# mahfuzalhasan/WaveFormer

Hardware: AMD Instinct MI355X
Metric: 128³×4 volumes/sec fwd (1/2/4/8 MI355X) + Dice Δ vs reference (higher is better)
Workload: dtype bf16x3; 1 GPU; MultiscaleTransformer (WaveFormer encoder) forward, 128^3x4 crops; global_batch=8, per_gpu_batch=8, precision=bf16x3, parallelism=replicas x1 (no data-path collective), hip_graph=True

## Files before the change

include/waveformer_hip.h:

```cpp
#ifndef WAVEFORMER_HIP_H
#define WAVEFORMER_HIP_H

#include <stdint.h>

#ifdef __cplusplus
extern "C" {
#endif

#define WF_ABI_VERSION 20

enum { WF_PREC_BF16 = 0, WF_PREC_BF16X3 = 1, WF_PREC_FP16 = 2 };

enum {
  WF_OK = 0,
  WF_E_SHAPE = -1,
  WF_E_NULLPTR = -2,
  WF_E_LAUNCH = -3
};

int wf_abi_version(void);
const char* wf_last_error(void);


int wf_cast_f32_to_bf16(const float* in, uint16_t* out, int64_t n, void* stream);

int wf_split_f32_to_bf16x2(const float* in, uint16_t* out, int64_t n, void* stream);

int wf_split_f32_to_bf16x2_multi(const int64_t* table_dev, int64_t n, int64_t total,
                                 void* stream);

int wf_cast_f32_to_f16x2(const float* in, uint16_t* out, int64_t n, void* stream);
int wf_cast_f32_to_f16x2_multi(const int64_t* table_dev, int64_t n, int64_t total,
                               void* stream);

int wf_debug_poison_lds(int64_t blocks, int lds_bytes, void* stream);

int wf_patch_embed_fwd(const float* x, const float* w, const float* bias, float* out,
                       int64_t B, int64_t Cin, int64_t Cout, int64_t D, int64_t H, int64_t W,
                       void* stream);
int wf_patch_embed_ll_fwd(const float* x, const float* w, const float* bias, float* out,
                          const float* ln_w, const float* ln_b, float ln_eps, float* ll,
                          int64_t B, int64_t Cin, int64_t Cout, int64_t D, int64_t H, int64_t W,
                          void* stream);

int wf_dwt3d_haar_fwd(const float* x, const float* ln_w, const float* ln_b, float ln_eps,
                      float* bands, int64_t B, int64_t C, int64_t D, int64_t H, int64_t W,
                      void* stream);
int wf_dwt3d_haar_fwd_ll(const float* x, const float* ln_w, const float* ln_b, float ln_eps,
                         float* ll, int64_t B, int64_t C, int64_t D, int64_t H, int64_t W,
                         void* stream);

int wf_idwt3d_haar(const float* ll, int64_t ll_bstride, const float* const* det,
                   const int64_t* det_s, int levels, float* out, int64_t out_bstride,
                   int64_t B, int64_t C, int64_t d, int64_t h, int64_t w, void* stream);
int wf_idwt3d_haar_cl(const float* ll, int64_t ll_bstride, int64_t ll_cstride,
                      int64_t ll_pstride, const float* const* det, const int64_t* det_s,
                      int levels, float* out, int64_t out_bstride, int64_t ldo, int64_t B,
                      int64_t C, int64_t d, int64_t h, int64_t w, void* stream);

int wf_idwt3d_haar_cl_cat(const float* ll, int64_t ll_bstride, int64_t ll_cstride,
                          int64_t ll_pstride, const float* const* det, const int64_t* det_s,
                          int levels, const float* skip, int64_t skip_bstride, int64_t skip_ld,
                          float* out, int64_t out_bstride, int64_t ldo, int64_t B, int64_t C,
                          int64_t d, int64_t h, int64_t w, void* stream);

int wf_copy_cl(const float* src, int64_t lds, float* dst, int64_t ldd, int64_t P, int64_t C,
               void* stream);
int wf_subvoxel_scatter_cl(const float* g, const float* bias, float* dst, int64_t ldd,
                           int64_t B, int64_t C, int64_t d, int64_t h, int64_t w, void* stream);
int wf_convtranspose2_cl(const float* x, const uint16_t* w_bf16x2, const float* bias, float* out,
                         int64_t ldo, int64_t B, int64_t Cin, int64_t Cout, int64_t d, int64_t h,
                         int64_t w, int precision, void* stream);

int wf_dwt3d_fwd(const float* x, float* bands, int64_t P, int64_t D, int64_t H, int64_t W,
                 const float* dec_lo, const float* dec_hi, int taps, void* stream);

int wf_idwt3d_level(const float* const* coef, const int64_t* coef_strides, int64_t B, int64_t C,
                    int64_t n_z, int64_t n_y, int64_t n_x, const float* rec_lo,
                    const float* rec_hi, int taps, float* out, int64_t out_bstride,
                    int64_t out_cstride, void* stream);

int wf_dwt3d_bwd(const float* gbands, float* dx, int64_t P, int64_t D, int64_t H, int64_t W,
                 const float* dec_lo, const float* dec_hi, int taps, void* stream);

int wf_idwt3d_level_bwd(const float* gout, int64_t gout_bstride, int64_t gout_cstride, int64_t B,
                        int64_t C, int64_t n_z, int64_t n_y, int64_t n_x, int extra_z,
                        int extra_y, int extra_x, const float* rec_lo, const float* rec_hi,
                        int taps, float* const* gcoef, const int64_t* gcoef_strides,
                        void* stream);

int64_t wf_conv3d_k3_packed_elems(int64_t Cin, int64_t Cout);
int wf_conv3d_k3_pack(const float* w, uint16_t* packed, int64_t Cin, int64_t Cout, void* stream);
int wf_conv3d_k3_pack_f16(const float* w, uint16_t* packed, int64_t Cin, int64_t Cout,
                          void* stream);
int64_t wf_conv3d_k3_workspace_bytes(int64_t B, int64_t Cin, int64_t Cout, int64_t D, int64_t H,
                                     int64_t W, int precision, int fp16_input);
int wf_conv3d_k3_fwd(const float* x, int64_t ldx, const uint16_t* w_packed, const float* bias,
                     float* out, int64_t ldo, double* stats_acc, void* workspace, int64_t B,
                     int64_t Cin, int64_t Cout, int64_t D, int64_t H, int64_t W, int precision,
                     void* stream);
int wf_conv3d_k3_fwd_xh(const uint16_t* x, int64_t ldx, const uint16_t* w_packed_f16,
                        const float* bias, float* out, int64_t ldo, double* stats_acc,
                        void* workspace, int64_t B, int64_t Cin, int64_t Cout, int64_t D,
                        int64_t H, int64_t W, void* stream);

int64_t wf_conv3d_k3_wgrad_workspace_bytes(int64_t B, int64_t Cin, int64_t Cout, int64_t D,
                                           int64_t H, int64_t W);
int wf_conv3d_k3_wgrad(const float* x, int64_t ldx, const float* dy, int64_t ldg, float* dw,
                       int accumulate, void* workspace, int64_t B, int64_t Cin, int64_t Cout,
                       int64_t D, int64_t H, int64_t W, void* stream);

int64_t wf_instnorm_workspace_bytes(int64_t B, int64_t C);
int wf_instnorm_stats_cl(const float* x, int64_t ldx, int64_t B, int64_t C, int64_t P, float eps,
                         float* stats, void* workspace, void* stream);
int wf_instnorm_finalize(const double* acc, float* stats, int64_t B, int64_t C, int64_t P,
                         float eps, void* stream);
int wf_norm_act_cl(const float* a, int64_t lda, const float* stats_a, const float* r, int64_t ldr,
                   const float* stats_r, float* out, int64_t ldo, int64_t B, int64_t C, int64_t P,
                   float slope, void* stream);
int wf_norm_act_h_cl(const float* a, int64_t lda, const float* stats_a, uint16_t* out,
                     int64_t ldo, int64_t B, int64_t C, int64_t P, float slope, void* stream);

int wf_moments_cl(const float* x, int64_t ldx, int64_t B, int64_t K, int64_t P, double* acc,
                  void* stream);
int wf_norm_act_lin_cl(const float* a, int64_t lda, const float* stats_a, const float* x,
                       int64_t ldx, int64_t K, const float* wfold, const float* bfold,
                       float* out, int64_t ldo, int64_t B, int64_t C, int64_t P, float slope,
                       void* stream);

int64_t wf_hf_refine_workspace_bytes(int64_t B, int64_t C);
int wf_hf_refine_fwd(const float* const* details, int64_t ldb, const float* dw_w,
                     const float* dw_b, const float* in_w, const float* in_b, float eps,
                     const float* pw_w, const float* pw_b, int sigmoid, float* out,
                     void* workspace, int64_t B, int64_t C, int64_t D, int64_t H, int64_t W,
                     void* stream);

int64_t wf_norm_act_bwd_workspace_bytes(int64_t B, int64_t C);
int wf_norm_act_bwd_cl(const float* dy, int64_t ldd, const float* y, int64_t ldy,
                       const float* a, int64_t lda, const float* stats_a, const float* r,
                       int64_t ldr, const float* stats_r, float* da, int64_t ldda, float* dr,
                       int64_t lddr, int64_t B, int64_t C, int64_t P, float slope,
                       void* workspace, void* stream);

int wf_upsample_trilinear_cl(const float* in, float* out, int64_t B, int64_t C, int64_t d,
                             int64_t h, int64_t w, int64_t D, int64_t H, int64_t W,
                             int align_corners, void* stream);
int wf_upsample_trilinear_add_cl(const float* in, float* out, int64_t B, int64_t C, int64_t d,
                                 int64_t h, int64_t w, int64_t D, int64_t H, int64_t W,
                                 int align_corners, void* stream);
int wf_upsample_dwconv3d_stats_cl(const float* in, const float* w, const float* bias, float* out,
                                  double* stats_acc, int64_t B, int64_t C, int64_t d, int64_t h,
                                  int64_t wd, int64_t D, int64_t H, int64_t W, int align_corners,
                                  void* stream);
int wf_conv1x1_head_cl(const float* x, int64_t ldx, const float* weight, const float* bias,
                       float* out, int64_t B, int64_t K, int64_t N, int64_t P, void* stream);
int wf_linear_smallk_fwd(const float* x, int64_t ldx, const float* w, const float* bias,
                         float* y, int64_t ldy, int64_t M, int64_t K, int64_t N, void* stream);
int wf_dwconv3d_stats_cl(const float* in, const float* w, const float* bias, float* out,
                         double* stats_acc, int64_t B, int64_t C, int64_t D, int64_t H,
                         int64_t W, void* stream);

int wf_resample_trilinear_cf(const float* in, int64_t ldc, int64_t C, int64_t d, int64_t h,
                             int64_t w, int64_t D, int64_t H, int64_t W, int align_corners,
                             void* out, int out_f16, void* stream);

int wf_linear_fwd(const float* x, const uint16_t* w_bf16x2, const float* bias, float* out,
                  int64_t M, int64_t K, int64_t N, int gelu_in, int precision, void* stream);

int wf_window_attention_fwd_table(const float* x, const float* ln_w, const float* ln_b,
                                  float ln_eps, const uint16_t* wqkv_bf16x2, const float* bqkv,
                                  const float* table, const uint16_t* wproj_bf16x2,
                                  const float* bproj, float* out, void* workspace, int64_t B,
                                  int64_t C, int64_t D1, int64_t H1, int64_t W1, int64_t ws,
                                  int64_t heads, float scale, int precision, void* stream);

int wf_rel_pos_bias(const float* table, const int64_t* index, float* bias, int64_t N,
                    int64_t heads, int64_t table_rows, void* stream);

int64_t wf_window_attention_workspace_bytes(int64_t B, int64_t C, int64_t D1, int64_t H1,
                                            int64_t W1, int precision);
int wf_window_attention_fwd(const float* x, const float* ln_w, const float* ln_b, float ln_eps,
                            const uint16_t* wqkv_bf16x2, const float* bqkv,
                            const float* bias, const uint16_t* wproj_bf16x2, const float* bproj,
                            float* out, void* workspace, int64_t B, int64_t C, int64_t D1,
                            int64_t H1, int64_t W1, int64_t ws, int64_t heads, float scale,
                            int precision, void* stream);

int64_t wf_window_attention_levels_workspace_bytes(const int64_t* dhw, int nlev, int64_t B,
                                                   int64_t C, int precision);
int wf_window_attention_fwd_levels(const float* const* x, const int64_t* dhw, int nlev,
                                   const uint16_t* wqkv_bf16x2, const float* bqkv,
                                   const float* table, const uint16_t* wproj_bf16x2,
                                   const float* bproj, float* out, void* workspace, int64_t B,
                                   int64_t C, int64_t heads, float scale, int precision,
                                   void* stream);

int wf_msfuse_fwd(const float* const* src, const int64_t* src_dhw, int nsrc,
                  const float* shortcut, const float* branch_scale, float* out, float* stats,
                  float ln_eps, int64_t B, int64_t C, int64_t D, int64_t H, int64_t W,
                  void* stream);

int64_t wf_ccf_ffn_workspace_bytes(int64_t B, int64_t C, int64_t hidden, int64_t D, int64_t H,
                                   int64_t W, int precision);
int wf_ccf_ffn_fwd(const float* xh, const float* stats, const float* n2_w, const float* n2_b,
                   const uint16_t* pw_bf16x2, const float* pw_b, const float* ln1_w,
                   const float* ln1_b, float eps1, const float* dw_w, const float* dw_b,
                   const float* ln2_w, const float* ln2_b, float eps2,
                   const uint16_t* fc_bf16x2, const float* fc_b, const float* branch_scale,
                   float* out, void* workspace,
                   int64_t B, int64_t C, int64_t hidden, int64_t D, int64_t H, int64_t W,
                   int precision, void* stream);
int wf_ccf_ffn_stage(int stage, const float* xh, const float* stats, const float* n2_w,
                     const float* n2_b, const uint16_t* pw_bf16x2, const float* pw_b,
                     const float* ln1_w, const float* ln1_b, float eps1, const float* dw_w,
                     const float* dw_b, const float* ln2_w, const float* ln2_b, float eps2,
                     const uint16_t* fc_bf16x2, const float* fc_b, const float* branch_scale,
                     float* out, void* workspace, int64_t B, int64_t C, int64_t hidden,
                     int64_t D, int64_t H, int64_t W, int precision, void* stream);

int wf_patch_merging_fwd(const float* x, const float* ln_w, const float* ln_b, float eps,
                         const uint16_t* red_bf16x2, int v2, float* out, int64_t B, int64_t C,
                         int64_t D, int64_t H, int64_t W, int precision, void* stream);

int wf_proj_out_fwd(const float* x, float* out, int normalize, float eps, int64_t B,
                    int64_t C, int64_t S, void* stream);
int wf_proj_out_cl_fwd(const float* x, float* out, float eps, int64_t M, int64_t C, void* stream);

int wf_importance_map(int mode, const float* sigma_scale, float* out, int64_t rd, int64_t rh,
                      int64_t rw, void* stream);

int wf_sliding_window_stitch(const float* patches, int64_t world, int64_t slots_per_round,
                             const float* importance_map, const int64_t* starts,
                             const int64_t* nwin, float* out, int64_t B, int64_t C, int64_t D,
                             int64_t H, int64_t W, int64_t rd, int64_t rh, int64_t rw,
                             void* stream);

int wf_sliding_window_stitch_partial(const float* patches, int64_t world, int64_t rank,
                                     const float* importance_map, const int64_t* starts,
                                     const int64_t* nwin, float* out, int64_t B, int64_t C,
                                     int64_t D, int64_t H, int64_t W, int64_t rd, int64_t rh,
                                     int64_t rw, void* stream);
int wf_sliding_window_normalize(const float* num, float* out, int64_t B, int64_t C, int64_t D,
                                int64_t H, int64_t W, void* stream);

int wf_tta_merge(const float* pred, const int* flips, int npass, float* out, int64_t C,
                 int64_t D, int64_t H, int64_t W, void* stream);


int wf_window_attention_fwd_train(const float* x, const float* ln_w, const float* ln_b,
                                  float ln_eps, const uint16_t* wqkv_bf16x2, const float* bqkv,
                                  const float* bias, const uint16_t* wproj_bf16x2,
                                  const float* bproj, float* out, void* workspace, float* lse,
                                  int64_t B, int64_t C, int64_t D1, int64_t H1, int64_t W1,
                                  int64_t ws, int64_t heads, float scale, int precision,
                                  void* stream);

int64_t wf_window_attention_bwd_workspace_bytes(int64_t B, int64_t C, int64_t D1, int64_t H1,
                                                int64_t W1, int64_t ws, int64_t heads);
int wf_window_attention_bwd_core(const float* qkv, const float* o, const float* dout,
                                 const float* bias, const float* lse, float* dqkv, float* dbias,
                                 void* workspace, int64_t B, int64_t C, int64_t D1, int64_t H1,
                                 int64_t W1, int64_t ws, int64_t heads, float scale,
                                 void* stream);

int64_t wf_gemm_tn_workspace_bytes(int64_t M, int64_t N, int64_t K);
int wf_gemm_tn(const float* a, int64_t lda, const float* b, int64_t ldb, float* c, int64_t ldc,
               int accumulate, void* workspace, int64_t M, int64_t N, int64_t K, void* stream);

int wf_rel_pos_bias_bwd(const float* dbias, const int64_t* perm, const int64_t* offsets,
                        float* dtable, int64_t N, int64_t heads, int64_t table_rows,
                        void* stream);

int64_t wf_colsum_parts(int64_t R);
int wf_colsum(const float* in, int64_t R, int64_t N, const float* row_scale,
              int64_t rows_per_scale, float* partials, float* out, void* stream);

int wf_ln_act_fwd(const float* x, const float* w, const float* b, float eps, int gelu, float* y,
                  int64_t M, int64_t N, void* stream);
int64_t wf_ln_bwd_workspace_floats(int64_t M, int64_t N);
int wf_ln_act_bwd(const float* x, const float* w, const float* b, float eps, int gelu,
                  const float* dy, const float* dadd, float* dx, float* partials, float* dw,
                  float* db, int64_t M, int64_t N, void* stream);

int wf_dwt3d_haar_bwd(const float* const* dband, const int64_t* strides, float* dx, int64_t B,
                      int64_t C, int64_t D, int64_t H, int64_t W, void* stream);

int wf_haar_analysis_ncdhw(const float* in, int64_t in_bstride, int64_t in_cstride, float* ll,
                           float* const* det, const int64_t* det_strides, int64_t B, int64_t C,
                           int64_t d, int64_t h, int64_t w, void* stream);

int wf_interp_adjoint_axis_ac(const float* in, float* out, int64_t outer, int64_t Lout,
                              int64_t Lin, int64_t inner, void* stream);
int wf_interp_adjoint_axis(const float* in, float* out, int64_t outer, int64_t Lout,
                           int64_t Lin, int64_t inner, const float* outer_scale,
                           int64_t outer_per_scale, void* stream);

int wf_dwconv3d_cl(const float* in, const float* w, const float* bias, int flip, float* out,
                   int64_t B, int64_t C, int64_t D, int64_t H, int64_t W, void* stream);
int64_t wf_dwconv_wgrad_ws_floats(int64_t B, int64_t C, int64_t D, int64_t H, int64_t W);
int wf_dwconv3d_wgrad(const float* dy, const float* x, float* partials, float* dw, int64_t B,
                      int64_t C, int64_t D, int64_t H, int64_t W, void* stream);

int wf_patch_merging_gather(const float* x, int v2, float* merged, int64_t B, int64_t C,
                            int64_t D, int64_t H, int64_t W, void* stream);
int wf_patch_merging_scatter(const float* dmerged, int v2, float* dx, int64_t B, int64_t C,
                             int64_t D, int64_t H, int64_t W, void* stream);

int wf_patchify(float* x, float* rows, int dir, int64_t B, int64_t Cin, int64_t D, int64_t H,
                int64_t W, void* stream);

int wf_transpose_cs(const float* in, float* out, int64_t B, int64_t C, int64_t S, void* stream);

#ifdef __cplusplus
}
#endif
#endif
```

waveformer_amd/_lib.py:

```python
from __future__ import annotations

import ctypes
import os
import threading

_HERE = os.path.dirname(os.path.abspath(__file__))
LIB_PATH = os.environ.get("WAVEFORMER_HIP_LIB", os.path.join(_HERE, "libwaveformer_hip.so"))

_P = ctypes.c_void_p
_I64 = ctypes.c_int64
_I = ctypes.c_int
_F = ctypes.c_float

SIGNATURES = {
    "wf_abi_version": (_I, []),
    "wf_last_error": (ctypes.c_char_p, []),
    "wf_cast_f32_to_bf16": (_I, [_P, _P, _I64, _P]),
    "wf_split_f32_to_bf16x2": (_I, [_P, _P, _I64, _P]),
    "wf_split_f32_to_bf16x2_multi": (_I, [_P, _I64, _I64, _P]),
    "wf_cast_f32_to_f16x2": (_I, [_P, _P, _I64, _P]),
    "wf_cast_f32_to_f16x2_multi": (_I, [_P, _I64, _I64, _P]),
    "wf_debug_poison_lds": (_I, [_I64, _I, _P]),
    "wf_patch_embed_ll_fwd": (_I, [_P, _P, _P, _P, _P, _P, _F, _P, _I64, _I64, _I64, _I64, _I64,
                                   _I64, _P]),
    "wf_patch_embed_fwd": (_I, [_P, _P, _P, _P, _I64, _I64, _I64, _I64, _I64, _I64, _P]),
    "wf_dwt3d_haar_fwd": (_I, [_P, _P, _P, _F, _P, _I64, _I64, _I64, _I64, _I64, _P]),
    "wf_dwt3d_haar_fwd_ll": (_I, [_P, _P, _P, _F, _P, _I64, _I64, _I64, _I64, _I64, _P]),
    "wf_idwt3d_haar": (_I, [_P, _I64, _P, _P, _I, _P, _I64, _I64, _I64, _I64, _I64, _I64, _P]),
    "wf_idwt3d_haar_cl": (_I, [_P, _I64, _I64, _I64, _P, _P, _I, _P, _I64, _I64, _I64, _I64,
                               _I64, _I64, _I64, _P]),
    "wf_idwt3d_haar_cl_cat": (_I, [_P, _I64, _I64, _I64, _P, _P, _I, _P, _I64, _I64, _P, _I64,
                                   _I64, _I64, _I64, _I64, _I64, _I64, _P]),
    "wf_copy_cl": (_I, [_P, _I64, _P, _I64, _I64, _I64, _P]),
    "wf_subvoxel_scatter_cl": (_I, [_P, _P, _P, _I64, _I64, _I64, _I64, _I64, _I64, _P]),
    "wf_convtranspose2_cl": (_I, [_P, _P, _P, _P, _I64, _I64, _I64, _I64, _I64, _I64, _I64, _I, _P]),
    "wf_moments_cl": (_I, [_P, _I64, _I64, _I64, _I64, _P, _P]),
    "wf_conv3d_k3_fwd_xh": (_I, [_P, _I64, _P, _P, _P, _I64, _P, _P, _I64, _I64, _I64, _I64, _I64,
                                 _I64, _P]),
    "wf_conv3d_k3_workspace_bytes": (_I64, [_I64, _I64, _I64, _I64, _I64, _I64, _I, _I]),
    "wf_norm_act_h_cl": (_I, [_P, _I64, _P, _P, _I64, _I64, _I64, _I64, _F, _P]),
    "wf_upsample_trilinear_add_cl": (_I, [_P, _P, _I64, _I64, _I64, _I64, _I64, _I64, _I64, _I64, _I, _P]),
    "wf_conv1x1_head_cl": (_I, [_P, _I64, _P, _P, _P, _I64, _I64, _I64, _I64, _P]),
    "wf_linear_smallk_fwd": (_I, [_P, _I64, _P, _P, _P, _I64, _I64, _I64, _I64, _P]),
    "wf_dwconv3d_stats_cl": (_I, [_P, _P, _P, _P, _P, _I64, _I64, _I64, _I64, _I64, _P]),
    "wf_norm_act_lin_cl": (_I, [_P, _I64, _P, _P, _I64, _I64, _P, _P, _P, _I64, _I64, _I64, _I64, _F, _P]),
    "wf_dwt3d_fwd": (_I, [_P, _P, _I64, _I64, _I64, _I64, _P, _P, _I, _P]),
    "wf_idwt3d_level": (_I, [_P, _P, _I64, _I64, _I64, _I64, _I64, _P, _P, _I, _P, _I64, _I64,
                             _P]),
    "wf_dwt3d_bwd": (_I, [_P, _P, _I64, _I64, _I64, _I64, _P, _P, _I, _P]),
    "wf_idwt3d_level_bwd": (_I, [_P, _I64, _I64, _I64, _I64, _I64, _I64, _I64, _I, _I, _I, _P,
                                 _P, _I, _P, _P, _P]),
    "wf_conv3d_k3_packed_elems": (_I64, [_I64, _I64]),
    "wf_conv3d_k3_pack": (_I, [_P, _P, _I64, _I64, _P]),
    "wf_conv3d_k3_pack_f16": (_I, [_P, _P, _I64, _I64, _P]),
    "wf_conv3d_k3_fwd": (_I, [_P, _I64, _P, _P, _P, _I64, _P, _P, _I64, _I64, _I64, _I64,
                              _I64, _I64, _I, _P]),
    "wf_instnorm_finalize": (_I, [_P, _P, _I64, _I64, _I64, _F, _P]),
    "wf_instnorm_workspace_bytes": (_I64, [_I64, _I64]),
    "wf_instnorm_stats_cl": (_I, [_P, _I64, _I64, _I64, _I64, _F, _P, _P, _P]),
    "wf_resample_trilinear_cf": (_I, [_P, _I64, _I64, _I64, _I64, _I64, _I64, _I64, _I64, _I,
                                      _P, _I, _P]),
    "wf_conv3d_k3_wgrad_workspace_bytes": (_I64, [_I64] * 6),
    "wf_conv3d_k3_wgrad": (_I, [_P, _I64, _P, _I64, _P, _I, _P, _I64, _I64, _I64, _I64, _I64,
                                _I64, _P]),
    "wf_norm_act_bwd_workspace_bytes": (_I64, [_I64, _I64]),
    "wf_norm_act_bwd_cl": (_I, [_P, _I64, _P, _I64, _P, _I64, _P, _P, _I64, _P, _P, _I64, _P, _I64,
                                _I64, _I64, _I64, _F, _P, _P]),
    "wf_hf_refine_workspace_bytes": (_I64, [_I64, _I64]),
    "wf_hf_refine_fwd": (_I, [_P, _I64, _P, _P, _P, _P, _F, _P, _P, _I, _P, _P, _I64, _I64,
                              _I64, _I64, _I64, _P]),
    "wf_norm_act_cl": (_I, [_P, _I64, _P, _P, _I64, _P, _P, _I64, _I64, _I64, _I64, _F, _P]),
    "wf_upsample_trilinear_cl": (_I, [_P, _P, _I64, _I64, _I64, _I64, _I64, _I64, _I64, _I64,
                                      _I, _P]),
    "wf_linear_fwd": (_I, [_P, _P, _P, _P, _I64, _I64, _I64, _I, _I, _P]),
    "wf_window_attention_fwd_table": (_I, [_P, _P, _P, _F, _P, _P, _P, _P, _P, _P, _P,
                                           _I64, _I64, _I64, _I64, _I64, _I64, _I64, _F, _I,
                                           _P]),
    "wf_rel_pos_bias": (_I, [_P, _P, _P, _I64, _I64, _I64, _P]),
    "wf_window_attention_workspace_bytes": (_I64, [_I64, _I64, _I64, _I64, _I64, _I]),
    "wf_window_attention_fwd": (_I, [_P, _P, _P, _F, _P, _P, _P, _P, _P, _P, _P,
                                     _I64, _I64, _I64, _I64, _I64, _I64, _I64, _F, _I, _P]),
    "wf_window_attention_levels_workspace_bytes": (_I64, [_P, _I, _I64, _I64, _I]),
    "wf_window_attention_fwd_levels": (_I, [_P, _P, _I, _P, _P, _P, _P, _P, _P, _P, _I64, _I64,
                                            _I64, _F, _I, _P]),
    "wf_msfuse_fwd": (_I, [_P, _P, _I, _P, _P, _P, _P, _F, _I64, _I64, _I64, _I64, _I64, _P]),
    "wf_ccf_ffn_workspace_bytes": (_I64, [_I64, _I64, _I64, _I64, _I64, _I64, _I]),
    "wf_ccf_ffn_fwd": (_I, [_P, _P, _P, _P, _P, _P, _P, _P, _F, _P, _P, _P, _P, _F, _P, _P,
                            _P, _P, _P, _I64, _I64, _I64, _I64, _I64, _I64, _I, _P]),
    "wf_ccf_ffn_stage": (_I, [_I, _P, _P, _P, _P, _P, _P, _P, _P, _F, _P, _P, _P, _P, _F, _P,
                              _P, _P, _P, _P, _I64, _I64, _I64, _I64, _I64, _I64, _I, _P]),
    "wf_patch_merging_fwd": (_I, [_P, _P, _P, _F, _P, _I, _P, _I64, _I64, _I64, _I64, _I64,
                                  _I, _P]),
    "wf_proj_out_fwd": (_I, [_P, _P, _I, _F, _I64, _I64, _I64, _P]),
    "wf_proj_out_cl_fwd": (_I, [_P, _P, _F, _I64, _I64, _P]),
    "wf_upsample_dwconv3d_stats_cl": (_I, [_P, _P, _P, _P, _P] + [_I64] * 8 + [_I, _P]),
    "wf_importance_map": (_I, [_I, _P, _P, _I64, _I64, _I64, _P]),
    "wf_sliding_window_stitch": (_I, [_P, _I64, _I64, _P, _P, _P, _P, _I64, _I64, _I64, _I64,
                                      _I64, _I64, _I64, _I64, _P]),
    "wf_tta_merge": (_I, [_P, _P, _I, _P, _I64, _I64, _I64, _I64, _P]),
    "wf_sliding_window_stitch_partial": (_I, [_P, _I64, _I64, _P, _P, _P, _P, _I64, _I64,
                                              _I64, _I64, _I64, _I64, _I64, _I64, _P]),
    "wf_sliding_window_normalize": (_I, [_P, _P, _I64, _I64, _I64, _I64, _I64, _P]),
    "wf_window_attention_fwd_train": (_I, [_P, _P, _P, _F, _P, _P, _P, _P, _P, _P, _P, _P,
                                           _I64, _I64, _I64, _I64, _I64, _I64, _I64, _F, _I,
                                           _P]),
    "wf_window_attention_bwd_workspace_bytes": (_I64, [_I64, _I64, _I64, _I64, _I64, _I64,
                                                       _I64]),
    "wf_window_attention_bwd_core": (_I, [_P, _P, _P, _P, _P, _P, _P, _P, _I64, _I64, _I64,
                                          _I64, _I64, _I64, _I64, _F, _P]),
    "wf_rel_pos_bias_bwd": (_I, [_P, _P, _P, _P, _I64, _I64, _I64, _P]),
    "wf_gemm_tn_workspace_bytes": (_I64, [_I64, _I64, _I64]),
    "wf_gemm_tn": (_I, [_P, _I64, _P, _I64, _P, _I64, _I, _P, _I64, _I64, _I64, _P]),
    "wf_colsum_parts": (_I64, [_I64]),
    "wf_colsum": (_I, [_P, _I64, _I64, _P, _I64, _P, _P, _P]),
    "wf_ln_act_fwd": (_I, [_P, _P, _P, _F, _I, _P, _I64, _I64, _P]),
    "wf_ln_bwd_workspace_floats": (_I64, [_I64, _I64]),
    "wf_ln_act_bwd": (_I, [_P, _P, _P, _F, _I, _P, _P, _P, _P, _P, _P, _I64, _I64, _P]),
    "wf_dwt3d_haar_bwd": (_I, [_P, _P, _P, _I64, _I64, _I64, _I64, _I64, _P]),
    "wf_haar_analysis_ncdhw": (_I, [_P, _I64, _I64, _P, _P, _P, _I64, _I64, _I64, _I64, _I64,
                                    _P]),
    "wf_interp_adjoint_axis": (_I, [_P, _P, _I64, _I64, _I64, _I64, _P, _I64, _P]),
    "wf_interp_adjoint_axis_ac": (_I, [_P, _P, _I64, _I64, _I64, _I64, _P]),
    "wf_dwconv3d_cl": (_I, [_P, _P, _P, _I, _P, _I64, _I64, _I64, _I64, _I64, _P]),
    "wf_dwconv_wgrad_ws_floats": (_I64, [_I64] * 5),
    "wf_dwconv3d_wgrad": (_I, [_P, _P, _P, _P, _I64, _I64, _I64, _I64, _I64, _P]),
    "wf_patch_merging_gather": (_I, [_P, _I, _P, _I64, _I64, _I64, _I64, _I64, _P]),
    "wf_patch_merging_scatter": (_I, [_P, _I, _P, _I64, _I64, _I64, _I64, _I64, _P]),
    "wf_patchify": (_I, [_P, _P, _I, _I64, _I64, _I64, _I64, _I64, _P]),
    "wf_transpose_cs": (_I, [_P, _P, _I64, _I64, _I64, _P]),
}

ABI_VERSION = 20
_lock = threading.Lock()
_lib = None
_err = None


class LibraryMissing(RuntimeError):
    pass


def load(path: str | None = None):
    global _lib, _err
    with _lock:
        if _lib is not None:
            return _lib
        p = path or LIB_PATH
        if not os.path.exists(p):
            _err = f"{p} not found: build it with `python -c 'import __graft_entry__ as g; g.build()'`"
            raise LibraryMissing(_err)
        lib = ctypes.CDLL(p)
        for name, (res, args) in SIGNATURES.items():
            fn = getattr(lib, name)
            fn.restype = res
            fn.argtypes = args
        ver = lib.wf_abi_version()
        if ver != ABI_VERSION:
            raise LibraryMissing(f"{p}: ABI version {ver}, expected {ABI_VERSION} (rebuild)")
        _lib = lib
        return _lib


def call(name: str, *args) -> None:
    lib = load()
    rc = getattr(lib, name)(*args)
    if rc != 0:
        msg = lib.wf_last_error().decode(errors="replace")
        raise RuntimeError(f"{name} failed ({rc}): {msg}")


def query(name: str, *args) -> int:
    return int(getattr(load(), name)(*args))
```

waveformer_amd/csrc/attention.hip:

```cpp
#include "attn_levels.hpp"
#include "kernels.hpp"

namespace wf {

constexpr int kQB = 64;

__device__ __forceinline__ void attn_block(int gx, int heads, int& qb, int& h, int64_t& bw) {
  const int64_t L = blockIdx.x, nb = gridDim.x;
  const int64_t xcd = L & 7, q8 = nb >> 3, r8 = nb & 7;
  int64_t t = (xcd < r8 ? xcd * (q8 + 1) : r8 * (q8 + 1) + (xcd - r8) * q8) + (L >> 3);
  qb = (int)(t % gx);
  t /= gx;
  h = (int)(t % heads);
  bw = t / heads;
}

template <int P>
__device__ __forceinline__ void load8_split(const void* base, int64_t off, bf16x8& hi,
                                            bf16x8& lo) {
  if (store32(P)) {
    const f32x4* p = reinterpret_cast<const f32x4*>(reinterpret_cast<const float*>(base) + off);
    const f32x4 a = p[0], b = p[1];
    const float v[8] = {a.x, a.y, a.z, a.w, b.x, b.y, b.z, b.w};
#pragma unroll
    for (int j = 0; j < 8; ++j) {
      const uint16_t h = op_cvt<P>(v[j]);
      hi[j] = (short)h;
      lo[j] = op_lo<P>(v[j], h);
    }
  } else {
    hi = *reinterpret_cast<const bf16x8*>(reinterpret_cast<const uint16_t*>(base) + off);
  }
}

template <int HD, int KT, int P>
__global__ __launch_bounds__(256) void attn_core_kernel(const void* __restrict__ qkv,
                                                        const float* __restrict__ bias,
                                                        void* __restrict__ out,
                                                        float* __restrict__ lse, int N,
                                                        int heads, float scale_log2) {
  constexpr bool SPLIT = P == PREC_SPLIT;
  constexpr int NC = HD / 16;
  constexpr int NKT = KT / 16;
  constexpr int KS = HD + 4, VS = KT + 4;
  constexpr int NB = SPLIT ? 2 : 1;
  __shared__ __attribute__((aligned(16))) uint16_t Ks[NB][KT * KS];
  __shared__ __attribute__((aligned(16))) uint16_t Vt[NB][HD * VS];

  const int tid = threadIdx.x, lane = tid & 63, wid = tid >> 6;
  int qb, h;
  int64_t bw;
  attn_block((N + kQB - 1) / kQB, heads, qb, h, bw);
  const int C = heads * HD;
  const int64_t row0 = bw * N;
  const int ld = 3 * C;
  const int q = qb * kQB + wid * 16 + (lane & 15);
  const bool qv = q < N;
  const int g4 = 4 * (lane >> 4);

  bf16x4 qf[NC], qfl[NC];
#pragma unroll
  for (int c = 0; c < NC; ++c) {
    qf[c] = bf16x4{0, 0, 0, 0};
    qfl[c] = bf16x4{0, 0, 0, 0};
    if (!qv) continue;
    const int64_t off = (row0 + q) * ld + h * HD + c * 16 + g4;
    if (store32(P)) {
      const f32x4 v = *reinterpret_cast<const f32x4*>(reinterpret_cast<const float*>(qkv) + off);
#pragma unroll
      for (int j = 0; j < 4; ++j) {
        const uint16_t hh = op_cvt<P>(v[j]);
        qf[c][j] = (short)hh;
        qfl[c][j] = op_lo<P>(v[j], hh);
      }
    } else {
      qf[c] = *reinterpret_cast<const bf16x4*>(reinterpret_cast<const uint16_t*>(qkv) + off);
    }
  }
  f32x4 o[NC];
#pragma unroll
  for (int c = 0; c < NC; ++c) o[c] = f32x4{0, 0, 0, 0};
  float mrun = -INFINITY, lrun = 0.f;
  const float* brow = bias + ((int64_t)h * N + (qv ? q : 0)) * N;

  for (int k0 = 0; k0 < N; k0 += KT) {
    __syncthreads();
    for (int it = tid; it < KT * (HD / 8); it += 256) {
      const int kr = it / (HD / 8), ch = it % (HD / 8);
      const int key = k0 + kr;
      bf16x8 kh = {0, 0, 0, 0, 0, 0, 0, 0}, kl = kh, vh = kh, vl = kh;
      if (key < N) {
        const int64_t off = (row0 + key) * ld + h * HD + ch * 8;
        load8_split<P>(qkv, off + C, kh, kl);
        load8_split<P>(qkv, off + 2 * C, vh, vl);
      }
      *reinterpret_cast<bf16x8*>(&Ks[0][kr * KS + ch * 8]) = kh;
      if (SPLIT) *reinterpret_cast<bf16x8*>(&Ks[NB - 1][kr * KS + ch * 8]) = kl;
#pragma unroll
      for (int j = 0; j < 8; ++j) {
        Vt[0][(ch * 8 + j) * VS + kr] = (uint16_t)vh[j];
        if (SPLIT) Vt[NB - 1][(ch * 8 + j) * VS + kr] = (uint16_t)vl[j];
      }
    }
    __syncthreads();

    f32x4 s[NKT];
#pragma unroll
    for (int kt = 0; kt < NKT; ++kt) {
      s[kt] = f32x4{0, 0, 0, 0};
#pragma unroll
      for (int c = 0; c < NC; ++c) {
        const int ko = (kt * 16 + (lane & 15)) * KS + c * 16 + g4;
        const bf16x4 a = *reinterpret_cast<const bf16x4*>(&Ks[0][ko]);
        if (SPLIT) {
          const bf16x4 al = *reinterpret_cast<const bf16x4*>(&Ks[NB - 1][ko]);
          s[kt] = mma16<P>(al, qf[c], s[kt]);
          s[kt] = mma16<P>(a, qfl[c], s[kt]);
        }
        s[kt] = mma16<P>(a, qf[c], s[kt]);
      }
    }
    float tmax = -INFINITY;
#pragma unroll
    for (int kt = 0; kt < NKT; ++kt) {
      const int kb = k0 + kt * 16 + g4;
      f32x4 bv;
      if (kb + 3 < N) {
        bv = *reinterpret_cast<const f32x4*>(brow + kb) * 1.4426950408889634f;
      } else {
        bv.x = kb + 0 < N ? brow[kb + 0] : 0.f;
        bv.y = kb + 1 < N ? brow[kb + 1] : 0.f;
        bv.z = kb + 2 < N ? brow[kb + 2] : 0.f;
        bv.w = kb + 3 < N ? brow[kb + 3] : 0.f;
        bv *= 1.4426950408889634f;
      }
#pragma unroll
      for (int i = 0; i < 4; ++i) {
        float t = s[kt][i] * scale_log2 + bv[i];
        t = (kb + i < N) ? t : -INFINITY;
        s[kt][i] = t;
        tmax = fmaxf(tmax, t);
      }
    }
    tmax = fmaxf(tmax, __shfl_xor(tmax, 16, 64));
    tmax = fmaxf(tmax, __shfl_xor(tmax, 32, 64));
    const float mnew = fmaxf(mrun, tmax);
    const float alpha = __builtin_amdgcn_exp2f(mrun - mnew);
    mrun = mnew;
    float psum = 0.f;
    bf16x4 pf[NKT], pfl[NKT];
#pragma unroll
    for (int kt = 0; kt < NKT; ++kt) {
#pragma unroll
      for (int i = 0; i < 4; ++i) {
        const float p = __builtin_amdgcn_exp2f(s[kt][i] - mnew);
        psum += p;
        const uint16_t ph = op_cvt<P>(p);
        pf[kt][i] = (short)ph;
        pfl[kt][i] = op_lo<P>(p, ph);
      }
    }
    lrun = lrun * alpha + psum;
#pragma unroll
    for (int c = 0; c < NC; ++c) {
      o[c] *= alpha;
#pragma unroll
      for (int kt = 0; kt < NKT; ++kt) {
        const int vo = (c * 16 + (lane & 15)) * VS + kt * 16 + g4;
        const bf16x4 a = *reinterpret_cast<const bf16x4*>(&Vt[0][vo]);
        if (SPLIT) {
          const bf16x4 al = *reinterpret_cast<const bf16x4*>(&Vt[NB - 1][vo]);
          o[c] = mma16<P>(al, pf[kt], o[c]);
          o[c] = mma16<P>(a, pfl[kt], o[c]);
        }
        o[c] = mma16<P>(a, pf[kt], o[c]);
      }
    }
  }
  lrun = xsum16(lrun);
  lrun = xsum32(lrun);
  if (lse && qv && lane < 16) lse[(bw * heads + h) * N + q] = mrun + __log2f(lrun);
  if (qv) {
    const float inv = 1.f / lrun;
    const int64_t off = (row0 + q) * C + h * HD + g4;
#pragma unroll
    for (int c = 0; c < NC; ++c) {
      if (store32(P)) {
        *reinterpret_cast<f32x4*>(reinterpret_cast<float*>(out) + off + c * 16) = o[c] * inv;
      } else {
        bf16x4 r;
#pragma unroll
        for (int i = 0; i < 4; ++i) r[i] = (short)f2bf(o[c][i] * inv);
        *reinterpret_cast<bf16x4*>(reinterpret_cast<uint16_t*>(out) + off + c * 16) = r;
      }
    }
  }
}

template <int P>
__device__ __forceinline__ void load8_split_scaled(const void* base, int64_t off, float sc,
                                                   bf16x8& hi, bf16x8& lo) {
  if (store32(P)) {
    const f32x4* p = reinterpret_cast<const f32x4*>(reinterpret_cast<const float*>(base) + off);
    const f32x4 a = p[0] * sc, b = p[1] * sc;
    const float v[8] = {a.x, a.y, a.z, a.w, b.x, b.y, b.z, b.w};
#pragma unroll
    for (int j = 0; j < 8; ++j) {
      const uint16_t h = op_cvt<P>(v[j]);
      hi[j] = (short)h;
      lo[j] = op_lo<P>(v[j], h);
    }
  } else {
    const bf16x8 r = *reinterpret_cast<const bf16x8*>(reinterpret_cast<const uint16_t*>(base) + off);
#pragma unroll
    for (int j = 0; j < 8; ++j) hi[j] = (short)f2bf(bf2f((uint16_t)r[j]) * sc);
  }
}

__device__ __forceinline__ int kswz(int row) {
  return (0x78 >> (2 * ((row >> 2) & 3))) & 3;
}

namespace tbl {
constexpr int N = 512, HD = 16;
constexpr int TBLN = 547;
constexpr int KS = 32;
constexpr int VB = HD * 4 + 4;
constexpr int VQ = (N / 4) * VB;
constexpr int TQ_BYTES = TBLN * 16;
constexpr float kTau = 16.0f;
}

template <int P, int NQ>
__device__ __forceinline__ void attn_tbl_tiles(const void* __restrict__ qkv, void* __restrict__ out,
                                               const f32x4* tq, const uint16_t* Ks,
                                               const uint16_t* Vq, int64_t row0, int q0, int h,
                                               int heads, int nsub, float scale_log2) {
  using namespace tbl;
  constexpr bool SPLIT = P == PREC_SPLIT;
  constexpr bool VSUM = SPLIT;
  const int lane = threadIdx.x & 63, wid = threadIdx.x >> 6;
  const int l15 = lane & 15, g4 = lane >> 4;
  const int C = heads * HD, ld = 3 * C;
  const int kch = 8 * (g4 ^ kswz(l15));
  const bf16x8 z8 = {0, 0, 0, 0, 0, 0, 0, 0};
  const short one = (short)op_cvt<P>(1.0f);
  const bf16x8 ones = bf16x8{one, one, one, one, one, one, one, one};
  for (int st = wid; st < nsub; st += 8 * NQ) {
    int qq[NQ], rbq[NQ];
    bf16x8 b1[NQ], b2[NQ];
    f32x4 o[NQ], l4[NQ];
    float mrun[NQ];
#pragma unroll
    for (int u = 0; u < NQ; ++u) {
      const int q = q0 + (st + 8 * u) * 16 + l15;
      qq[u] = q;
      bf16x8 hi = z8, lo = z8;
      load8_split_scaled<P>(qkv, (row0 + q) * ld + h * HD + 8 * (g4 & 1), scale_log2, hi, lo);
      b1[u] = hi;
      b2[u] = (SPLIT && g4 < 2) ? lo : z8;
      const int qz = q >> 6, qy = (q >> 3) & 7, qx = q & 7;
      rbq[u] = (TBLN - 1) - ((qz + 7) * 23 + (qy + 7) * 15 + (qx + 7)) +
               ((g4 >> 1) * 15 + 4 * (g4 & 1));
      o[u] = f32x4{0.f, 0.f, 0.f, 0.f};
      l4[u] = f32x4{0.f, 0.f, 0.f, 0.f};
      mrun[u] = -INFINITY;
    }
#pragma clang loop unroll_count(NQ == 1 ? 2 : 1)
    for (int t = 0; t < 8; ++t) {
      f32x4 s[NQ][4];
#pragma unroll
      for (int kt = 0; kt < 4; ++kt) {
        const bf16x8 a = *reinterpret_cast<const bf16x8*>(&Ks[(t * 64 + kt * 16 + l15) * KS + kch]);
#pragma unroll
        for (int u = 0; u < NQ; ++u) {
          s[u][kt] = mma32<P>(a, b1[u], tq[rbq[u] + 23 * t + 30 * kt]);
          if (SPLIT) s[u][kt] = mma32<P>(a, b2[u], s[u][kt]);
        }
      }
      float lmax[NQ];
      bool big = false;
#pragma unroll
      for (int u = 0; u < NQ; ++u) {
        lmax[u] = s[u][0][0];
#pragma unroll
        for (int kt = 0; kt < 4; ++kt)
#pragma unroll
          for (int i = (kt == 0 ? 1 : 0); i < 4; ++i) lmax[u] = fmaxf(lmax[u], s[u][kt][i]);
        big = big || lmax[u] > mrun[u] + kTau;
      }
      if (__builtin_amdgcn_ballot_w64(big) != 0) {
#pragma unroll
        for (int u = 0; u < NQ; ++u) {
          float tmax = fmaxf(mrun[u], lmax[u]);
          tmax = fmaxf(tmax, __shfl_xor(tmax, 16, 64));
          tmax = fmaxf(tmax, __shfl_xor(tmax, 32, 64));
          const float alpha = __builtin_amdgcn_exp2f(mrun[u] - tmax);
          mrun[u] = tmax;
          o[u] *= alpha;
          l4[u] *= alpha;
        }
      }
      uint32_t ph[NQ][4][2], pl[NQ][4][2];
#pragma unroll
      for (int u = 0; u < NQ; ++u)
#pragma unroll
        for (int kt = 0; kt < 4; ++kt)
#pragma unroll
          for (int i = 0; i < 4; i += 2) {
            const float e0 = __builtin_amdgcn_exp2f(s[u][kt][i] - mrun[u]);
            const float e1 = __builtin_amdgcn_exp2f(s[u][kt][i + 1] - mrun[u]);
            if (VSUM) l4[u][0] += e0 + e1;
            split_pair<P>(e0, e1, ph[u][kt][i >> 1], pl[u][kt][i >> 1]);
          }
#pragma unroll
      for (int j = 0; j < 2; ++j) {
        const int o1 = (16 * t + 8 * j + g4) * VB + l15 * 4;
        const int o2 = (16 * t + 8 * j + 4 + g4) * VB + l15 * 4;
        const bf16x4 v1 = *reinterpret_cast<const bf16x4*>(&Vq[o1]);
        const bf16x4 v2 = *reinterpret_cast<const bf16x4*>(&Vq[o2]);
        const bf16x8 vh = bf16x8{v1[0], v1[1], v1[2], v1[3], v2[0], v2[1], v2[2], v2[3]};
        bf16x8 vl = z8;
        if (SPLIT) {
          const bf16x4 w1 = *reinterpret_cast<const bf16x4*>(&Vq[VQ + o1]);
          const bf16x4 w2 = *reinterpret_cast<const bf16x4*>(&Vq[VQ + o2]);
          vl = bf16x8{w1[0], w1[1], w1[2], w1[3], w2[0], w2[1], w2[2], w2[3]};
        }
#pragma unroll
        for (int u = 0; u < NQ; ++u) {
          const bf16x8 pb = __builtin_bit_cast(
              bf16x8, u32x4{ph[u][2 * j][0], ph[u][2 * j][1], ph[u][2 * j + 1][0], ph[u][2 * j + 1][1]});
          if (SPLIT) {
            const bf16x8 plb = __builtin_bit_cast(
                bf16x8, u32x4{pl[u][2 * j][0], pl[u][2 * j][1], pl[u][2 * j + 1][0], pl[u][2 * j + 1][1]});
            o[u] = mma32<P>(vl, pb, o[u]);
            o[u] = mma32<P>(vh, plb, o[u]);
            if (!VSUM) l4[u] = mma32<P>(ones, plb, l4[u]);
          }
          o[u] = mma32<P>(vh, pb, o[u]);
          if (!VSUM) l4[u] = mma32<P>(ones, pb, l4[u]);
        }
      }
    }
#pragma unroll
    for (int u = 0; u < NQ; ++u) {
      if (VSUM) {
        l4[u][0] += __shfl_xor(l4[u][0], 16, 64);
        l4[u][0] += __shfl_xor(l4[u][0], 32, 64);
      }
      const float inv = 1.f / l4[u][0];
      const int64_t off = (row0 + qq[u]) * C + h * HD + 4 * g4;
      if (store32(P)) {
        *reinterpret_cast<f32x4*>(reinterpret_cast<float*>(out) + off) = o[u] * inv;
      } else {
        bf16x4 r;
#pragma unroll
        for (int i = 0; i < 4; ++i) r[i] = (short)f2bf(o[u][i] * inv);
        *reinterpret_cast<bf16x4*>(reinterpret_cast<uint16_t*>(out) + off) = r;
      }
    }
  }
}

template <int P>
__global__ __launch_bounds__(512, 2) void attn_tbl_kernel(const void* __restrict__ qkv,
                                                          const float* __restrict__ table,
                                                          void* __restrict__ out, int heads,
                                                          int qsplit, float scale_log2,
                                                          int64_t pair_end) {
  using namespace tbl;
  constexpr bool SPLIT = P == PREC_SPLIT;
  __shared__ __attribute__((aligned(16))) uint8_t lds_tbl[TQ_BYTES + N * KS * 2 + 2 * VQ * 2];
  f32x4* tq = reinterpret_cast<f32x4*>(lds_tbl);
  uint16_t* Ks = reinterpret_cast<uint16_t*>(lds_tbl + TQ_BYTES);
  uint16_t* Vq = Ks + N * KS;
  const int tid = threadIdx.x;
  int qs, h;
  int64_t bw;
  attn_block(qsplit, heads, qs, h, bw);
  const int C = heads * HD, ld = 3 * C;
  const int64_t row0 = bw * N;
  const bf16x8 z8 = {0, 0, 0, 0, 0, 0, 0, 0};

  for (int i = tid; i < TBLN; i += 512) {
    const float v = table[(int64_t)i * heads + h] * 1.4426950408889634f;
    const int j = TBLN - 1 - i;
#pragma unroll
    for (int c = 0; c < 4; ++c)
      if (j - c >= 0) reinterpret_cast<float*>(&tq[j - c])[c] = v;
    if (j >= TBLN - 3)
      for (int c = TBLN - j; c < 4; ++c) reinterpret_cast<float*>(&tq[j])[c] = 0.f;
  }
  for (int it = tid; it < N * 2; it += 512) {
    const int key = it >> 1, ch = it & 1, sw = kswz(key);
    bf16x8 hi = z8, lo = z8;
    load8_split<P>(qkv, (row0 + key) * ld + C + h * HD + ch * 8, hi, lo);
    *reinterpret_cast<bf16x8*>(&Ks[key * KS + 8 * (ch ^ sw)]) = hi;
    *reinterpret_cast<bf16x8*>(&Ks[key * KS + 8 * ((2 + ch) ^ sw)]) = SPLIT ? lo : z8;
  }
  for (int it = tid; it < (N / 4) * 2; it += 512) {
    const int k4 = it >> 1, ch = it & 1;
    bf16x8 vh[4], vl[4];
#pragma unroll
    for (int r = 0; r < 4; ++r) {
      vh[r] = z8;
      vl[r] = z8;
      load8_split<P>(qkv, (row0 + 4 * k4 + r) * ld + 2 * C + h * HD + ch * 8, vh[r], vl[r]);
    }
#pragma unroll
    for (int j = 0; j < 8; ++j) {
      const int o = k4 * VB + (ch * 8 + j) * 4;
      *reinterpret_cast<bf16x4*>(&Vq[o]) = bf16x4{vh[0][j], vh[1][j], vh[2][j], vh[3][j]};
      if (SPLIT) *reinterpret_cast<bf16x4*>(&Vq[VQ + o]) = bf16x4{vl[0][j], vl[1][j], vl[2][j], vl[3][j]};
    }
  }
  __syncthreads();

  const int nsub = N / 16 / qsplit;
  const int q0 = qs * (N / qsplit);
  if (nsub >= 16 && bw < pair_end)
    attn_tbl_tiles<P, 2>(qkv, out, tq, Ks, Vq, row0, q0, h, heads, nsub, scale_log2);
  else
    attn_tbl_tiles<P, 1>(qkv, out, tq, Ks, Vq, row0, q0, h, heads, nsub, scale_log2);
}

bool attn_tbl_pair_loop(int64_t wh) { return wh >= 256; }

int launch_attn_core(const void* qkv, const float* bias, void* out, float* lse, int64_t Bw,
                     int N, int heads, int hd, float scale, int prec, hipStream_t s,
                     int table_ws, int64_t pair_windows) {
  if (Bw <= 0) return WF_OK;
  const int64_t nblk = cdiv(N, kQB) * heads * Bw;
  if (nblk > 0x7fffffff) return fail(WF_E_SHAPE, "attention: too many (window, head) tiles");
  dim3 grid((unsigned)nblk);
  const float sl2 = scale * 1.4426950408889634f;
  const bool split = prec == PREC_SPLIT;
  const bool f16 = prec == PREC_FP16;
  if (!valid_prec(prec)) return fail(WF_E_SHAPE, "attention: unknown precision");
  if (table_ws) {
    if (table_ws != 8 || hd != 16 || N != 512)
      return fail(WF_E_SHAPE, "attention (table bias): implemented for ws = 8, head_dim = 16");
    if (lse) return fail(WF_E_SHAPE, "attention (table bias): inference only, no log-sum-exp");
    const int64_t wh = Bw * heads;
    const int qsplit = wh >= 512 ? 1 : (attn_tbl_pair_loop(wh) ? 2 : 4);
    const dim3 g1((unsigned)(wh * qsplit));
    auto k = split ? attn_tbl_kernel<PREC_SPLIT>
                   : (f16 ? attn_tbl_kernel<PREC_FP16> : attn_tbl_kernel<PREC_BF16>);
    const int64_t pair_end = pair_windows < 0 ? Bw : pair_windows;
    hipLaunchKernelGGL(k, g1, dim3(512), 0, s, qkv, bias, out, heads, qsplit, sl2, pair_end);
    return check_launch("attention core (table bias, window per workgroup)");
  }
#define ATTN_HD_CASE(HDV)                                                                  \
  case HDV: {                                                                              \
    auto k = split ? attn_core_kernel<HDV, (HDV >= 192 ? 32 : 64), PREC_SPLIT>             \
                   : (f16 ? attn_core_kernel<HDV, 64, PREC_FP16>                           \
                          : attn_core_kernel<HDV, 64, PREC_BF16>);                         \
    hipLaunchKernelGGL(k, grid, dim3(256), 0, s, qkv, bias, out, lse, N, heads, sl2);      \
    break;                                                                                 \
  }
  switch (hd) {
    ATTN_HD_CASE(16)
    ATTN_HD_CASE(32)
    ATTN_HD_CASE(48)
    ATTN_HD_CASE(64)
    ATTN_HD_CASE(96)
    ATTN_HD_CASE(128)
    ATTN_HD_CASE(192)
    ATTN_HD_CASE(384)
    default:
      return fail(WF_E_SHAPE, "attention: head_dim must be one of 16,32,48,64,96,128,192,384");
  }
#undef ATTN_HD_CASE
  return check_launch("attention core");
}

__global__ void rel_pos_bias_kernel(const float* __restrict__ table, const int64_t* __restrict__ index,
                                    float* __restrict__ bias, int64_t NN, int heads) {
  const int64_t i = (int64_t)blockIdx.x * blockDim.x + threadIdx.x;
  if (i >= NN) return;
  const int64_t r = index[i];
  for (int h = 0; h < heads; ++h) bias[h * NN + i] = table[r * heads + h];
}

struct AttnWorkspace {
  int64_t ao, bytes;
};
static AttnWorkspace attn_workspace(int64_t rows, int64_t C, int prec) {
  const int64_t e = store32(prec) ? 4 : 2;
  const int64_t ao = align256(rows * 3 * C * e);
  return {ao, ao + align256(rows * C * e)};
}

static GemmArgs qkv_gemm_args(const float* x, const float* ln_w, const float* ln_b, float ln_eps,
                              const uint16_t* wqkv, const float* bqkv, void* qkv, int64_t rows,
                              int64_t B, int64_t C, int64_t D1, int64_t H1, int64_t W1,
                              int64_t ws, int prec) {
  GemmArgs g{};
  g.prec = prec;
  g.a_src = x;
  g.a_bf16 = 0;
  g.a_C = (int)C;
  g.a_nseg = 1;
  g.a_map = MAP_WINDOW;
  g.mB = (int)B;
  g.mD = (int)D1;
  g.mH = (int)H1;
  g.mW = (int)W1;
  g.mws = (int)ws;
  g.a_ln = ln_w ? LN_COMPUTE : LN_NONE;
  g.a_ln_w = ln_w;
  g.a_ln_b = ln_b;
  g.a_eps = ln_eps;
  g.w = wqkv;
  g.M = rows;
  g.N = (int)(3 * C);
  g.K = (int)C;
  g.epi = EPI_STORE;
  g.bias = bqkv;
  g.out = qkv;
  g.out_bf16 = !store32(prec);
  g.ldo = 3 * C;
  return g;
}

static GemmArgs proj_gemm_args(const void* ao, const uint16_t* wproj, const float* bproj,
                               float* out, int64_t rows, int64_t C, int prec) {
  GemmArgs p{};
  p.prec = prec;
  p.a_src = ao;
  p.a_bf16 = !store32(prec);
  p.a_C = (int)C;
  p.a_nseg = 1;
  p.a_map = MAP_IDENTITY;
  p.a_ln = LN_NONE;
  p.w = wproj;
  p.M = rows;
  p.N = (int)C;
  p.K = (int)C;
  p.epi = EPI_STORE;
  p.bias = bproj;
  p.out = out;
  p.out_bf16 = 0;
  p.ldo = C;
  return p;
}

}

using namespace wf;

extern "C" int wf_rel_pos_bias(const float* table, const int64_t* index, float* bias, int64_t N,
                               int64_t heads, int64_t table_rows, void* stream) {
  WF_REQUIRE(N >= 1 && heads >= 1 && table_rows >= 1, "empty bias");
  WF_REQUIRE_PTR(table);
  WF_REQUIRE_PTR(index);
  WF_REQUIRE_PTR(bias);
  const int64_t NN = N * N;
  hipLaunchKernelGGL(rel_pos_bias_kernel, dim3((unsigned)cdiv(NN, 256)), dim3(256), 0,
                     (hipStream_t)stream, table, index, bias, NN, (int)heads);
  return check_launch("wf_rel_pos_bias");
}

extern "C" int64_t wf_window_attention_workspace_bytes(int64_t B, int64_t C, int64_t D1,
                                                       int64_t H1, int64_t W1, int precision) {
  return attn_workspace(B * D1 * H1 * W1, C, precision).bytes;
}

static int window_attention_impl(const float* x, const float* ln_w, const float* ln_b,
                                 float ln_eps, const uint16_t* wqkv_bf16x2, const float* bqkv,
                                 const float* bias, int table_ws,
                                 const uint16_t* wproj_bf16x2, const float* bproj, float* out,
                                 void* workspace, float* lse, int64_t B, int64_t C, int64_t D1,
                                 int64_t H1, int64_t W1, int64_t ws, int64_t heads, float scale,
                                 int precision, void* stream) {
  WF_REQUIRE(B >= 1 && C >= 8 && C % 8 == 0, "C must be a positive multiple of 8");
  WF_REQUIRE(ws >= 1 && D1 % ws == 0 && H1 % ws == 0 && W1 % ws == 0,
             "the raster must tile into ws^3 windows (window_partition, wave_helper.py:459)");
  WF_REQUIRE(heads >= 1 && C % heads == 0, "dim must be divisible by num_heads");
  WF_REQUIRE(valid_prec(precision), "unknown precision");
  WF_REQUIRE_PTR(x);
  WF_REQUIRE_PTR(wqkv_bf16x2);
  WF_REQUIRE_PTR(bias);
  WF_REQUIRE_PTR(wproj_bf16x2);
  WF_REQUIRE_PTR(out);
  WF_REQUIRE_PTR(workspace);
  if (ln_w) WF_REQUIRE_PTR(ln_b);
  const int64_t N = ws * ws * ws;
  const int64_t rows = B * D1 * H1 * W1;
  const int64_t Bw = rows / N;
  hipStream_t s = (hipStream_t)stream;
  void* qkv = workspace;
  void* ao = reinterpret_cast<char*>(workspace) + attn_workspace(rows, C, precision).ao;
  int rc = launch_gemm(qkv_gemm_args(x, ln_w, ln_b, ln_eps, wqkv_bf16x2, bqkv, qkv, rows, B, C,
                                     D1, H1, W1, ws, precision),
                       s, "wf_window_attention_fwd(qkv)");
  if (rc) return rc;
  rc = launch_attn_core(qkv, bias, ao, lse, Bw, (int)N, (int)heads, (int)(C / heads), scale,
                        precision, s, table_ws);
  if (rc) return rc;
  return launch_gemm(proj_gemm_args(ao, wproj_bf16x2, bproj, out, rows, C, precision), s,
                     "wf_window_attention_fwd(proj)");
}

extern "C" int wf_window_attention_fwd_train(const float* x, const float* ln_w,
                                             const float* ln_b, float ln_eps,
                                             const uint16_t* wqkv_bf16x2, const float* bqkv,
                                             const float* bias, const uint16_t* wproj_bf16x2,
                                             const float* bproj, float* out, void* workspace,
                                             float* lse, int64_t B, int64_t C, int64_t D1,
                                             int64_t H1, int64_t W1, int64_t ws, int64_t heads,
                                             float scale, int precision, void* stream) {
  return window_attention_impl(x, ln_w, ln_b, ln_eps, wqkv_bf16x2, bqkv, bias, 0, wproj_bf16x2,
                               bproj, out, workspace, lse, B, C, D1, H1, W1, ws, heads, scale,
                               precision, stream);
}

extern "C" int wf_window_attention_fwd_table(const float* x, const float* ln_w,
                                             const float* ln_b, float ln_eps,
                                             const uint16_t* wqkv_bf16x2, const float* bqkv,
                                             const float* table, const uint16_t* wproj_bf16x2,
                                             const float* bproj, float* out, void* workspace,
                                             int64_t B, int64_t C, int64_t D1, int64_t H1,
                                             int64_t W1, int64_t ws, int64_t heads, float scale,
                                             int precision, void* stream) {
  WF_REQUIRE(ws == 8 && C == 16 * heads,
             "table-bias attention is implemented for window 8 and head_dim 16");
  return window_attention_impl(x, ln_w, ln_b, ln_eps, wqkv_bf16x2, bqkv, table, (int)ws,
                               wproj_bf16x2, bproj, out, workspace, nullptr, B, C, D1, H1, W1,
                               ws, heads, scale, precision, stream);
}

extern "C" int wf_window_attention_fwd(const float* x, const float* ln_w, const float* ln_b,
                                       float ln_eps, const uint16_t* wqkv_bf16x2,
                                       const float* bqkv, const float* bias,
                                       const uint16_t* wproj_bf16x2, const float* bproj,
                                       float* out, void* workspace, int64_t B, int64_t C,
                                       int64_t D1, int64_t H1, int64_t W1, int64_t ws,
                                       int64_t heads, float scale, int precision, void* stream) {
  return wf_window_attention_fwd_train(x, ln_w, ln_b, ln_eps, wqkv_bf16x2, bqkv, bias,
                                       wproj_bf16x2, bproj, out, workspace, nullptr, B, C, D1,
                                       H1, W1, ws, heads, scale, precision, stream);
}

extern "C" int64_t wf_window_attention_levels_workspace_bytes(const int64_t* dhw, int nlev,
                                                              int64_t B, int64_t C,
                                                              int precision) {
  AttnLevels L;
  if (attn_levels_plan(dhw, nlev, B, C, C / 16, L)) return WF_E_SHAPE;
  return attn_workspace(L.row0[nlev], C, precision).bytes;
}

extern "C" int wf_window_attention_fwd_levels(const float* const* x, const int64_t* dhw, int nlev,
                                              const uint16_t* wqkv_bf16x2, const float* bqkv,
                                              const float* table, const uint16_t* wproj_bf16x2,
                                              const float* bproj, float* out, void* workspace,
                                              int64_t B, int64_t C, int64_t heads, float scale,
                                              int precision, void* stream) {
  AttnLevels L;
  if (const char* why = attn_levels_plan(dhw, nlev, B, C, heads, L))
    return fail(WF_E_SHAPE, std::string(__func__) + ": " + why);
  WF_REQUIRE(valid_prec(precision), "unknown precision");
  WF_REQUIRE_PTR(x);
  for (int l = 0; l < nlev; ++l) {
    WF_REQUIRE_PTR(x[l]);
    WF_REQUIRE(reinterpret_cast<uintptr_t>(x[l]) % 16 == 0, "level sources must be 16-byte aligned");
  }
  WF_REQUIRE_PTR(wqkv_bf16x2);
  WF_REQUIRE_PTR(table);
  WF_REQUIRE_PTR(wproj_bf16x2);
  WF_REQUIRE_PTR(out);
  WF_REQUIRE_PTR(workspace);
  constexpr int64_t ws = kAttnLevelsWs, N = ws * ws * ws;
  const int64_t rows = L.row0[nlev];
  hipStream_t s = (hipStream_t)stream;
  void* qkv = workspace;
  void* ao = reinterpret_cast<char*>(workspace) + attn_workspace(rows, C, precision).ao;
  GemmArgs g = qkv_gemm_args(x[0], nullptr, nullptr, 0.f, wqkv_bf16x2, bqkv, qkv, rows, B, C, 0,
                             0, 0, ws, precision);
  g.a_map = MAP_LEVELS;
  for (int l = 0; l < WF_MAX_LEVELS; ++l) {
    const bool on = l < nlev;
    g.lv_src[l] = on ? x[l] : x[0];
    g.lv_row0[l] = on ? (int)L.row0[l] : 0x7fffffff;
    g.lv_D[l] = on ? L.D[l] : (int)ws;
    g.lv_H[l] = on ? L.H[l] : (int)ws;
    g.lv_W[l] = on ? L.W[l] : (int)ws;
  }
  int64_t pair_windows = 0;
  bool prefix = true;
  for (int l = 0; l < nlev; ++l) {
    const int64_t wl = (L.row0[l + 1] - L.row0[l]) / N;
    if (attn_tbl_pair_loop(wl * heads)) {
      prefix = prefix && pair_windows == L.row0[l] / N;
      pair_windows = L.row0[l + 1] / N;
    }
  }
  if (!prefix || (!try_launch_gemm_rows(g, s, true) && !try_launch_gemm_kc(g, s))) {
    for (int l = 0; l < nlev; ++l) {
      const int rc = window_attention_impl(x[l], nullptr, nullptr, 0.f, wqkv_bf16x2, bqkv, table,
                                           (int)ws, wproj_bf16x2, bproj, out + L.row0[l] * C,
                                           workspace, nullptr, B, C, L.D[l], L.H[l], L.W[l], ws,
                                           heads, scale, precision, stream);
      if (rc) return rc;
    }
    return WF_OK;
  }
  int rc = check_launch("wf_window_attention_fwd_levels(qkv)");
  if (rc) return rc;
  rc = launch_attn_core(qkv, table, ao, nullptr, rows / N, (int)N, (int)heads, 16, scale,
                        precision, s, (int)ws, pair_windows);
  if (rc) return rc;
  return launch_gemm(proj_gemm_args(ao, wproj_bf16x2, bproj, out, rows, C, precision), s,
                     "wf_window_attention_fwd_levels(proj)");
}
```

waveformer_amd/csrc/attn_levels.hpp:

```cpp
#pragma once
#include <stdint.h>

namespace wf {

constexpr int kAttnMaxLevels = 4;
constexpr int kAttnLevelsWs = 8;

struct AttnLevels {
  int nlev;
  int64_t row0[kAttnMaxLevels + 1];
  int D[kAttnMaxLevels], H[kAttnMaxLevels], W[kAttnMaxLevels];
};

inline const char* attn_levels_plan(const int64_t* dhw, int nlev, int64_t B, int64_t C,
                                    int64_t heads, AttnLevels& L) {
  if (nlev < 1 || nlev > kAttnMaxLevels) return "1 to 4 levels";
  if (dhw == nullptr) return "dhw is NULL";
  if (B < 1) return "B must be positive";
  if (heads < 1 || C != 16 * heads) return "table-bias attention needs head_dim 16 (C == 16 * heads)";
  L.nlev = nlev;
  L.row0[0] = 0;
  for (int l = 0; l < nlev; ++l) {
    const int64_t d = dhw[3 * l], h = dhw[3 * l + 1], w = dhw[3 * l + 2];
    if (d < kAttnLevelsWs || h < kAttnLevelsWs || w < kAttnLevelsWs || d % kAttnLevelsWs != 0 ||
        h % kAttnLevelsWs != 0 || w % kAttnLevelsWs != 0)
      return "every raster must tile into 8^3 windows (window_partition, wave_helper.py:459)";
    if (d > 0x7fffffff / h || d * h > 0x7fffffff / w || d * h * w > 0x7fffffff / B)
      return "a level has 2^31 rows or more";
    L.D[l] = (int)d;
    L.H[l] = (int)h;
    L.W[l] = (int)w;
    L.row0[l + 1] = L.row0[l] + B * d * h * w;
    if (L.row0[l + 1] > 0x7fffffff) return "2^31 rows or more";
  }
  return nullptr;
}

}
```

waveformer_amd/csrc/kernels.hpp:

```cpp
#pragma once
#include "wf_common.hpp"

namespace wf {

enum Prec { PREC_BF16 = 0, PREC_SPLIT = 1, PREC_FP16 = 2 };

typedef _Float16 f16x4 __attribute__((ext_vector_type(4)));
typedef _Float16 f16x8 __attribute__((ext_vector_type(8)));
__device__ __forceinline__ uint16_t f2h(float f) { return __builtin_bit_cast(uint16_t, (_Float16)f); }

template <int P>
__device__ __forceinline__ uint16_t op_cvt(float x) {
  if constexpr (P == PREC_FP16) return f2h(x);
  else return f2bf(x);
}
template <int P>
__device__ __forceinline__ short op_lo(float x, uint16_t hi) {
  if constexpr (P == PREC_SPLIT) return (short)f2bf(x - bf2f(hi));
  else return (short)0;
}
template <int P>
__device__ __forceinline__ f32x4 mma32(bf16x8 a, bf16x8 b, f32x4 c) {
  if constexpr (P == PREC_FP16)
    return __builtin_amdgcn_mfma_f32_16x16x32_f16(__builtin_bit_cast(f16x8, a),
                                                  __builtin_bit_cast(f16x8, b), c, 0, 0, 0);
  else return __builtin_amdgcn_mfma_f32_16x16x32_bf16(a, b, c, 0, 0, 0);
}
template <int P>
__device__ __forceinline__ f32x4 mma16(bf16x4 a, bf16x4 b, f32x4 c) {
  if constexpr (P == PREC_FP16)
    return __builtin_amdgcn_mfma_f32_16x16x16f16(__builtin_bit_cast(f16x4, a),
                                                 __builtin_bit_cast(f16x4, b), c, 0, 0, 0);
  else return __builtin_amdgcn_mfma_f32_16x16x16bf16_1k(a, b, c, 0, 0, 0);
}
template <int P>
__device__ __forceinline__ f32x4 mma3(f32x4 acc, const bf16x8& w_hi, const bf16x8& w_lo,
                                      const bf16x8& a_hi, const bf16x8& a_lo) {
  if constexpr (P == PREC_SPLIT) {
    acc = mma32<P>(w_hi, a_lo, acc);
    acc = mma32<P>(w_lo, a_hi, acc);
  }
  return mma32<P>(w_hi, a_hi, acc);
}
typedef __bf16 bf16v2 __attribute__((ext_vector_type(2)));
template <int P>
__device__ __forceinline__ void split_pair(float y0, float y1, uint32_t& hi, uint32_t& lo) {
  if constexpr (P == PREC_SPLIT) {
    uint32_t m0, m1;
    asm("s_mov_b32 %0, 0xbf80" : "=s"(m0));
    asm("s_mov_b32 %0, 0xbf800000" : "=s"(m1));
    const bf16v2 h = bf16v2{(__bf16)y0, (__bf16)y1};
    const float r0 = __builtin_amdgcn_fdot2_f32_bf16(h, __builtin_bit_cast(bf16v2, m0), y0, false);
    const float r1 = __builtin_amdgcn_fdot2_f32_bf16(h, __builtin_bit_cast(bf16v2, m1), y1, false);
    hi = __builtin_bit_cast(uint32_t, h);
    lo = __builtin_bit_cast(uint32_t, bf16v2{(__bf16)r0, (__bf16)r1});
  } else {
    hi = (uint32_t)op_cvt<P>(y0) | ((uint32_t)op_cvt<P>(y1) << 16);
    lo = 0;
  }
}
template <int P>
__device__ __forceinline__ void split4(f32x4 v, bf16x4& h, bf16x4& l) {
  uint32_t h0, h1, l0, l1;
  split_pair<P>(v[0], v[1], h0, l0);
  split_pair<P>(v[2], v[3], h1, l1);
  h = __builtin_bit_cast(bf16x4, u32x2{h0, h1});
  l = __builtin_bit_cast(bf16x4, u32x2{l0, l1});
}
template <int P>
__device__ __forceinline__ void split8(const float (&x)[8], bf16x8& h, bf16x8& l) {
  uint32_t hw[4], lw[4];
#pragma unroll
  for (int j = 0; j < 4; ++j) split_pair<P>(x[2 * j], x[2 * j + 1], hw[j], lw[j]);
  h = __builtin_bit_cast(bf16x8, u32x4{hw[0], hw[1], hw[2], hw[3]});
  l = __builtin_bit_cast(bf16x8, u32x4{lw[0], lw[1], lw[2], lw[3]});
}
__host__ __device__ constexpr bool store32(int p) { return p != PREC_BF16; }
inline bool valid_prec(int p) { return p == PREC_BF16 || p == PREC_SPLIT || p == PREC_FP16; }

enum RowMap { MAP_IDENTITY = 0, MAP_WINDOW = 1, MAP_MERGE = 2, MAP_LEVELS = 3 };
constexpr int WF_MAX_LEVELS = 4;
enum LnMode { LN_NONE = 0, LN_GIVEN = 1, LN_COMPUTE = 2, LN_PARTIAL = 3 };
enum EpiMode { EPI_STORE = 0, EPI_LN_GELU = 1, EPI_RESID = 2, EPI_SUBVOXEL = 3 };

struct GemmArgs {
  int prec;
  const void* a_src;
  int a_bf16;
  int a_C;
  int a_nseg;
  int a_map;
  int mB, mD, mH, mW, mws;
  int merge_code;
  int a_ln;
  const float* a_stats;
  int a_np;
  const float* a_ln_w;
  const float* a_ln_b;
  float a_eps;
  int a_gelu;
  const uint16_t* w;
  int64_t M;
  int N, K;
  int epi;
  const float* bias;
  void* out;
  int out_bf16;
  int64_t ldo;
  const float* e_ln_w;
  const float* e_ln_b;
  float e_eps;
  const float* r_x;
  const float* r_stats;
  const float* r_ln_w;
  const float* r_ln_b;
  const float* r_scale;
  int64_t rows_per_sample;
  float* o_pstats;
  float* kpart;
  int64_t kpart_bytes;
  int ksplit;
  const float* lv_src[WF_MAX_LEVELS];
  int lv_row0[WF_MAX_LEVELS];
  int lv_D[WF_MAX_LEVELS], lv_H[WF_MAX_LEVELS], lv_W[WF_MAX_LEVELS];
};

int launch_gemm(const GemmArgs& g, hipStream_t s, const char* who);
int gemm_kc_pick_nt(const GemmArgs& g);
int launch_instnorm_partial(const float* x, int64_t ldx, int64_t B, int64_t C, int64_t P,
                            double* acc, hipStream_t s);
int try_launch_gemm_rows(const GemmArgs& g, hipStream_t s, bool single_chunk_only);

int launch_attn_core(const void* qkv, const float* bias, void* out, float* lse, int64_t Bw,
                     int N, int heads, int hd, float scale, int prec, hipStream_t s,
                     int table_ws = 0, int64_t pair_windows = -1);
bool attn_tbl_pair_loop(int64_t wh);

int launch_dwconv_ln_gelu(const void* in, const float* w, const float* b, const float* ln_w,
                          const float* ln_b, float eps, void* out, int B, int Hd, int D, int H,
                          int W, int prec, hipStream_t s);
int launch_dwconv3d(const void* in, const float* w, const float* b, void* out, float* pstats,
                    int B, int Hd, int D, int H, int W, int prec, hipStream_t s,
                    double* cstats = nullptr, const float* ln1_stats = nullptr,
                    const float* ln1_w = nullptr, const float* ln1_b = nullptr, int flip = 0);
int launch_ln_stats_finalize(const float* pstats, int np, int group, float eps, float* out,
                             int64_t M, hipStream_t s);
constexpr int DW_STAT_GROUP = 32;
int try_launch_gemm_kc(const GemmArgs& g, hipStream_t s);
int try_launch_merge_resident(const GemmArgs& g, hipStream_t s);
int try_launch_pw2_resident(const GemmArgs& g, hipStream_t s);
int try_launch_gemm_lnw(const GemmArgs& g, hipStream_t s);
bool gemm_lnw_wide_shape(const GemmArgs& g);

}

#include "ffn_dwfc_common.hpp"
```

waveformer_amd/ops.py:

```python
from __future__ import annotations

import ctypes
import math
import os
import threading
import weakref
from typing import Dict, List, Optional, Sequence, Tuple

import torch

from . import _lib

DETAIL_KEYS = ("aad", "ada", "add", "daa", "dad", "dda", "ddd")


def _stream() -> int:
    return torch.cuda.current_stream().cuda_stream


def _ptr(t: Optional[torch.Tensor]) -> Optional[int]:
    return None if t is None else t.data_ptr()


def _check(t: torch.Tensor, name: str, dtype=torch.float32, contiguous=True) -> None:
    if not isinstance(t, torch.Tensor):
        raise TypeError(f"{name}: expected a tensor, got {type(t)}")
    if t.device.type != "cuda":
        raise RuntimeError(
            f"{name}: waveformer_amd kernels run on the GPU only (got a {t.device} tensor); "
            "move the module and inputs to cuda")
    if t.dtype != dtype:
        raise TypeError(f"{name}: expected {dtype}, got {t.dtype}")
    if contiguous and not t.is_contiguous():
        raise ValueError(f"{name}: expected a contiguous tensor")


PRECISIONS = {"bf16": 0, "bf16x3": 1, "fp16": 2}
FP16 = PRECISIONS["fp16"]
_precision = os.environ.get("WAVEFORMER_PRECISION", "bf16x3")
if _precision not in PRECISIONS:
    raise ValueError(f"WAVEFORMER_PRECISION={_precision!r}: expected one of {sorted(PRECISIONS)}")
_prec_tls = threading.local()


def set_precision(p: str) -> None:
    global _precision
    if p not in PRECISIONS:
        raise ValueError(f"precision must be one of {sorted(PRECISIONS)}, got {p!r}")
    _precision = p


def get_precision() -> str:
    o = getattr(_prec_tls, "override", None)
    return _precision if o is None else o


class precision:

    def __init__(self, p: str):
        if p not in PRECISIONS:
            raise ValueError(f"precision must be one of {sorted(PRECISIONS)}, got {p!r}")
        self.p = p

    def __enter__(self):
        self.prev = getattr(_prec_tls, "override", None)
        _prec_tls.override = self.p
        return self

    def __exit__(self, *exc):
        _prec_tls.override = self.prev


def _prec() -> int:
    return PRECISIONS[get_precision()]


def prec_id() -> int:
    return PRECISIONS[get_precision()]


FP16_SPLIT_OPS = frozenset({"attn", "skip_conv"})


def op_prec(kind: str) -> int:
    cur = get_precision()
    if cur == "fp16" and kind in FP16_SPLIT_OPS:
        return PRECISIONS["bf16x3"]
    return PRECISIONS[cur]


class op_precision(precision):

    def __init__(self, kind: str):
        self.kind = kind

    def __enter__(self):
        self.prev = getattr(_prec_tls, "override", None)
        cur = get_precision()
        self.p = "bf16x3" if op_prec(self.kind) != PRECISIONS[cur] else cur
        _prec_tls.override = self.p
        return self


class WeightArena:

    def __init__(self, params: Sequence[torch.Tensor], f16: bool = False):
        dev = params[0].device
        self.f16 = f16
        self.key = tuple((p.data_ptr(), p.numel()) for p in params)
        pre, dsts, off = [0], [], 0
        blocks = []
        for p in params:
            blocks.append(off)
            off += 2 * p.numel()
        self.buf = torch.empty(max(off, 8), dtype=torch.bfloat16, device=dev)
        self.views: Dict[int, torch.Tensor] = {}
        for p, o in zip(params, blocks):
            v = self.buf[o:o + 2 * p.numel()]
            self.views[p.data_ptr()] = v
            dsts.append(v.data_ptr())
            pre.append(pre[-1] + p.numel())
        self.n, self.total = len(params), pre[-1]
        table = pre + [p.data_ptr() for p in params] + dsts
        self.table = torch.tensor(table, dtype=torch.int64).to(dev)
        self.done: Optional[torch.cuda.Event] = None
        self.done_stream = None

    def refresh(self) -> None:
        cur = torch.cuda.current_stream(self.buf.device)
        if (self.done is not None and self.done_stream != cur.cuda_stream
                and not torch.cuda.is_current_stream_capturing()):
            cur.wait_event(self.done)
        _lib.call("wf_cast_f32_to_f16x2_multi" if self.f16 else "wf_split_f32_to_bf16x2_multi",
                  self.table.data_ptr(), self.n, self.total, cur.cuda_stream)

    def release(self) -> None:
        if torch.cuda.is_current_stream_capturing():
            return
        cur = torch.cuda.current_stream(self.buf.device)
        if self.done is None:
            self.done = torch.cuda.Event()
        self.done.record(cur)
        self.done_stream = cur.cuda_stream

    def retire(self) -> None:
        if self.done is not None:
            self.done.synchronize()


class _Scope:
    def __init__(self, arena: Optional[WeightArena]):
        self.arena = arena
        self.cache: Dict[tuple, torch.Tensor] = {}


_tls = threading.local()
_arena_lock = threading.Lock()
_ARENAS: "weakref.WeakKeyDictionary" = weakref.WeakKeyDictionary()


def arena_count(module: torch.nn.Module) -> int:
    with _arena_lock:
        return sum(len(per) for per in _ARENAS.get(module, {}).values())


def _cur_scope() -> Optional[_Scope]:
    return getattr(_tls, "scope", None)


def split_params(module: torch.nn.Module) -> List[torch.Tensor]:
    seen, out = set(), []
    for m in module.modules():
        fn = getattr(m, "_wf_split_params", None)
        if fn is None:
            continue
        for p in fn():
            if (p.is_cuda and p.dtype == torch.float32 and p.is_contiguous()
                    and p.numel() % 8 == 0 and p.data_ptr() not in seen):
                seen.add(p.data_ptr())
                out.append(p)
    return out


class weight_scope:

    def __init__(self, module: torch.nn.Module):
        self.module = module
        self.owner = False

    def __enter__(self):
        if _cur_scope() is not None:
            return self
        arena = None
        params = split_params(self.module)
        if params:
            train = torch.is_grad_enabled() and any(p.requires_grad for p in params)
            f16 = get_precision() == "fp16" and not train
            with _arena_lock:
                arenas = _ARENAS.get(self.module)
                if arenas is None:
                    arenas = {}
                    _ARENAS[self.module] = arenas
                for th in [t for t in arenas if not t.is_alive()]:
                    for old in arenas.pop(th).values():
                        old.retire()
                per = arenas.setdefault(threading.current_thread(), {})
                arena = per.get(f16)
                if arena is None or arena.key != tuple((p.data_ptr(), p.numel()) for p in params):
                    if arena is not None:
                        arena.retire()
                    arena = WeightArena(params, f16)
                    per[f16] = arena
            arena.refresh()
        _tls.scope = _Scope(arena)
        self.owner = True
        return self

    def __exit__(self, *exc):
        if self.owner:
            sc = _cur_scope()
            if sc is not None and sc.arena is not None:
                sc.arena.release()
            _tls.scope = None


def per_forward(key: tuple, make):
    sc = _cur_scope()
    if sc is None:
        return make()
    hit = sc.cache.get(key)
    if hit is None:
        v = make()
        ev = st = None
        if isinstance(v, torch.Tensor) and v.is_cuda:
            st = torch.cuda.current_stream(v.device)
            ev = torch.cuda.Event()
            ev.record(st)
        sc.cache[key] = (v, ev, st)
        return v
    v, ev, st = hit
    if ev is not None:
        cur = torch.cuda.current_stream(v.device)
        if cur != st:
            cur.wait_event(ev)
    return v


def split_weight(p: torch.Tensor, shape: Optional[Tuple[int, ...]] = None,
                 prec: Optional[int] = None) -> torch.Tensor:
    shp = (2,) + tuple(p.shape if shape is None else shape)
    f16 = (_prec() if prec is None else prec) == FP16
    sc = _cur_scope()
    if sc is not None and sc.arena is not None and sc.arena.f16 == f16:
        v = sc.arena.views.get(p.data_ptr())
        if v is not None and v.numel() == 2 * p.numel():
            return v.view(shp)

    def make():
        src = p.detach()
        _check(src, "weight")
        out = torch.empty(shp, dtype=torch.bfloat16, device=src.device)
        _lib.call("wf_cast_f32_to_f16x2" if f16 else "wf_split_f32_to_bf16x2", src.data_ptr(),
                  out.data_ptr(), src.numel(), _stream())
        return out
    return per_forward(("split", p.data_ptr(), shp, f16), make)


def patch_embed(x: torch.Tensor, weight: torch.Tensor, bias: Optional[torch.Tensor]) -> torch.Tensor:
    _check(x, "x")
    _check(weight, "weight")
    B, Cin, D2, H2, W2 = x.shape
    Cout = weight.shape[0]
    if tuple(weight.shape) != (Cout, Cin, 2, 2, 2):
        raise ValueError(f"patch_embed: weight {tuple(weight.shape)} is not ({Cout},{Cin},2,2,2)")
    if D2 % 2 or H2 % 2 or W2 % 2:
        raise ValueError("patch_embed: spatial sizes must be even (PatchEmbed pads otherwise)")
    if bias is not None:
        _check(bias, "bias")
    out = torch.empty((B, D2 // 2, H2 // 2, W2 // 2, Cout), dtype=torch.float32, device=x.device)
    _lib.call("wf_patch_embed_fwd", x.data_ptr(), weight.data_ptr(), _ptr(bias), out.data_ptr(),
              B, Cin, Cout, D2 // 2, H2 // 2, W2 // 2, _stream())
    return out


def patch_embed_ll(x: torch.Tensor, weight: torch.Tensor, bias: Optional[torch.Tensor],
                   ln: Tuple[torch.Tensor, torch.Tensor, float]
                   ) -> Optional[Tuple[torch.Tensor, torch.Tensor]]:
    B, Cin, D2, H2, W2 = x.shape
    Cout = weight.shape[0]
    D, H, W = D2 // 2, H2 // 2, W2 // 2
    if (Cout != 48 or Cin not in (1, 4) or tuple(weight.shape) != (Cout, Cin, 2, 2, 2)
            or D2 % 2 or H2 % 2 or W2 % 2 or D % 2 or H % 2 or W % 2 or W > 64
            or B * D * H * W * Cout >= 1 << 31):
        return None
    _check(x, "x")
    _check(weight, "weight")
    lw, lb, eps = ln
    _check(lw, "ln_w")
    _check(lb, "ln_b")
    if bias is not None:
        _check(bias, "bias")
    out = torch.empty((B, D, H, W, Cout), dtype=torch.float32, device=x.device)
    ll = torch.empty((B, D // 2, H // 2, W // 2, Cout), dtype=torch.float32, device=x.device)
    _lib.call("wf_patch_embed_ll_fwd", x.data_ptr(), weight.data_ptr(), _ptr(bias),
              out.data_ptr(), lw.data_ptr(), lb.data_ptr(), float(eps), ll.data_ptr(), B, Cin,
              Cout, D, H, W, _stream())
    return out, ll


def dwt3d_haar(x_cl: torch.Tensor, ln: Optional[Tuple[torch.Tensor, torch.Tensor, float]] = None
               ) -> torch.Tensor:
    _check(x_cl, "x")
    B, D, H, W, C = x_cl.shape
    bands = torch.empty((8, B, D // 2, H // 2, W // 2, C), dtype=torch.float32, device=x_cl.device)
    lw = lb = None
    eps = 0.0
    if ln is not None:
        lw, lb, eps = ln
        _check(lw, "ln_w")
        _check(lb, "ln_b")
    _lib.call("wf_dwt3d_haar_fwd", x_cl.data_ptr(), _ptr(lw), _ptr(lb), float(eps),
              bands.data_ptr(), B, C, D, H, W, _stream())
    return bands


def dwt3d_haar_ll(x_cl: torch.Tensor, ln: Optional[Tuple[torch.Tensor, torch.Tensor, float]] = None
                  ) -> torch.Tensor:
    _check(x_cl, "x")
    B, D, H, W, C = x_cl.shape
    ll = torch.empty((B, D // 2, H // 2, W // 2, C), dtype=torch.float32, device=x_cl.device)
    lw = lb = None
    eps = 0.0
    if ln is not None:
        lw, lb, eps = ln
        _check(lw, "ln_w")
        _check(lb, "ln_b")
    _lib.call("wf_dwt3d_haar_fwd_ll", x_cl.data_ptr(), _ptr(lw), _ptr(lb), float(eps),
              ll.data_ptr(), B, C, D, H, W, _stream())
    return ll


def bands_to_coeffs(bands) -> Tuple[torch.Tensor, Dict[str, torch.Tensor]]:
    ll = bands[0].permute(0, 4, 1, 2, 3)
    det = {k: bands[i + 1].permute(0, 4, 1, 2, 3) for i, k in enumerate(DETAIL_KEYS)}
    return ll, det


def idwt3d_haar(ll: torch.Tensor, details: Sequence[Dict[str, torch.Tensor]],
                out: Optional[torch.Tensor] = None,
                skip: Optional[torch.Tensor] = None) -> torch.Tensor:
    if ll.device.type != "cuda":
        raise RuntimeError("idwt3d_haar: GPU tensors only")
    if ll.dtype != torch.float32:
        raise TypeError("idwt3d_haar: float32 only")
    B, C, d, h, w = ll.shape
    ll_ld = cl_ld(ll)
    if ll_ld is None and ll.stride()[1:] != (d * h * w, h * w, w, 1):
        ll = ll.contiguous()
    L = len(details)
    if not 1 <= L <= 4:
        raise ValueError("idwt3d_haar: 1..4 detail levels supported")
    ptrs: List[int] = []
    strides: List[int] = []
    keep = []
    for l, dct in enumerate(details):
        s = 2 ** l
        exp = (B, C, d * s, h * s, w * s)
        ts = []
        for k in DETAIL_KEYS:
            t = dct[k]
            if tuple(t.shape) != exp:
                raise ValueError(f"idwt3d_haar: level {l} key {k} has shape {tuple(t.shape)}, expected {exp}")
            if t.device != ll.device or t.dtype != torch.float32:
                raise TypeError("idwt3d_haar: detail tensors must be float32 on the same GPU")
            ts.append(t)

        def pattern(t):
            st = t.stride()
            return (st[0], st[1], st[2], st[4]) if st[3] == exp[4] * st[4] else None

        pats = [pattern(t) for t in ts]
        if any(p is None for p in pats) or len(set(pats)) != 1:
            ts = [t.contiguous() for t in ts]
            pats = [pattern(t) for t in ts]
        keep.extend(ts)
        ptrs.extend(t.data_ptr() for t in ts)
        strides.extend(pats[0])
    Do, Ho, Wo = d * 2 ** L, h * 2 ** L, w * 2 ** L
    ldo = None
    if out is None:
        out = torch.empty((B, C, Do, Ho, Wo), dtype=torch.float32, device=ll.device)
    else:
        if out.shape[0] != B or out.shape[1] < C or tuple(out.shape[2:]) != (Do, Ho, Wo):
            raise ValueError(f"idwt3d_haar: out {tuple(out.shape)} does not fit ({B},{C},{Do},{Ho},{Wo})")
        ldo = cl_ld(out)
        if ldo is None and out.stride()[1:] != (Do * Ho * Wo, Ho * Wo, Wo, 1):
            raise ValueError("idwt3d_haar: out must be channel-last or contiguous inside each batch")
    arr = (ctypes.c_void_p * len(ptrs))(*ptrs)
    sarr = (ctypes.c_int64 * len(strides))(*strides)
    if ll_ld is not None and ldo is None:
        ll, ll_ld = ll.contiguous(), None
    if skip is not None and (out is None or out.shape[1] < 2 * C or tuple(skip.shape) != (B, C, Do, Ho, Wo)):
        raise ValueError("idwt3d_haar: skip must be (B, C, ...) of the output and out >= 2C channels")
    skip_ld = cl_ld(skip) if skip is not None else None
    fused = (skip is not None and ldo is not None and ll_ld is not None and skip_ld is not None
             and C % 4 == 0 and skip.device == out.device and skip.dtype == torch.float32
             and skip.stride(0) % 4 == 0 and skip.data_ptr() % 16 == 0
             and "WF_IDWT_SCALAR" not in os.environ)
    if fused:
        _lib.call("wf_idwt3d_haar_cl_cat", ll.data_ptr(), ll.stride(0), 1, ll_ld, arr, sarr, L,
                  skip.data_ptr(), skip.stride(0), skip_ld, out.data_ptr(), out.stride(0), ldo,
                  B, C, d, h, w, _stream())
    elif ldo is not None:
        ll_cs, ll_ps = (1, ll_ld) if ll_ld is not None else (d * h * w, 1)
        _lib.call("wf_idwt3d_haar_cl", ll.data_ptr(), ll.stride(0), ll_cs, ll_ps, arr, sarr, L,
                  out.data_ptr(), out.stride(0), ldo, B, C, d, h, w, _stream())
    else:
        _lib.call("wf_idwt3d_haar", ll.data_ptr(), ll.stride(0), arr, sarr, L, out.data_ptr(),
                  out.stride(0), B, C, d, h, w, _stream())
    if skip is not None and not fused:
        copy_cl(skip, out[:, C:2 * C])
    del keep
    return out


WAVELETS: Dict[str, Tuple[Tuple[float, ...], ...]] = {
    "db1": ((0.7071067811865476, 0.7071067811865476), (-0.7071067811865476, 0.7071067811865476),
            (0.7071067811865476, 0.7071067811865476), (0.7071067811865476, -0.7071067811865476)),
    "db2": ((-0.12940952255126037, 0.2241438680420134, 0.8365163037378079, 0.48296291314453416),
            (-0.48296291314453416, 0.8365163037378079, -0.2241438680420134, -0.12940952255126037),
            (0.48296291314453416, 0.8365163037378079, 0.2241438680420134, -0.12940952255126037),
            (-0.12940952255126037, -0.2241438680420134, 0.8365163037378079, -0.48296291314453416)),
    "db3": ((0.03522629188570953, -0.08544127388202666, -0.13501102001025458,
             0.45987750211849154, 0.8068915093110925, 0.33267055295008263),
            (-0.33267055295008263, 0.8068915093110925, -0.45987750211849154,
             -0.13501102001025458, 0.08544127388202666, 0.03522629188570953),
            (0.33267055295008263, 0.8068915093110925, 0.45987750211849154,
             -0.13501102001025458, -0.08544127388202666, 0.03522629188570953),
            (0.03522629188570953, 0.08544127388202666, -0.13501102001025458,
             -0.45987750211849154, 0.8068915093110925, -0.33267055295008263)),
    "db4": ((-0.010597401785069032, 0.0328830116668852, 0.030841381835560764,
             -0.18703481171909309, -0.027983769416859854, 0.6308807679298589,
             0.7148465705529157, 0.2303778133088965),
            (-0.2303778133088965, 0.7148465705529157, -0.6308807679298589,
             -0.027983769416859854, 0.18703481171909309, 0.030841381835560764,
             -0.0328830116668852, -0.010597401785069032),
            (0.2303778133088965, 0.7148465705529157, 0.6308807679298589,
             -0.027983769416859854, -0.18703481171909309, 0.030841381835560764,
             0.0328830116668852, -0.010597401785069032),
            (-0.010597401785069032, -0.0328830116668852, 0.030841381835560764,
             0.18703481171909309, -0.027983769416859854, -0.6308807679298589,
             0.7148465705529157, -0.2303778133088965)),
}
WAVELETS["haar"] = WAVELETS["db1"]


def wavelet_name(wavelet) -> str:
    name = str(getattr(wavelet, "name", wavelet))
    if name not in WAVELETS:
        raise NotImplementedError(f"wavelet {name!r}: only {sorted(WAVELETS)} are implemented")
    return name


def wavelet_taps(wavelet) -> int:
    return len(WAVELETS[wavelet_name(wavelet)][0])


def _filters(wavelet: str):
    name = wavelet_name(wavelet)
    return [(ctypes.c_float * len(f))(*f) for f in WAVELETS[name]], len(WAVELETS[name][0])


def dwt3d(x: torch.Tensor, wavelet: str) -> torch.Tensor:
    _check(x, "x", contiguous=False)
    if x.dim() != 5:
        raise ValueError(f"dwt3d: expected (B, C, D, H, W), got {tuple(x.shape)}")
    x = x.contiguous()
    (lo, hi, _, _), L = _filters(wavelet)
    B, C, D, H, W = x.shape
    bands = torch.empty((8, B, C, (D + L - 1) // 2, (H + L - 1) // 2, (W + L - 1) // 2),
                        dtype=torch.float32, device=x.device)
    _lib.call("wf_dwt3d_fwd", x.data_ptr(), bands.data_ptr(), B * C, D, H, W, lo, hi, L,
              _stream())
    return bands


def wavedec3(x: torch.Tensor, wavelet: str, level: int) -> List:
    if level < 1:
        raise ValueError("wavedec3: level must be >= 1")
    dets = []
    cur = x
    for _ in range(level):
        bands = dwt3d(cur, wavelet)
        dets.append({k: bands[i + 1] for i, k in enumerate(DETAIL_KEYS)})
        cur = bands[0]
    return [cur] + dets[::-1]


def waverec3(coeffs: Sequence, wavelet: str, out: Optional[torch.Tensor] = None) -> torch.Tensor:
    (_, _, rlo, rhi), L = _filters(wavelet)
    x = coeffs[0]
    _check(x, "LL", contiguous=False)
    nlev = len(coeffs) - 1
    if nlev < 1:
        raise ValueError("waverec3: need at least one detail level")
    for li, det in enumerate(coeffs[1:]):
        ts = [det[k] for k in DETAIL_KEYS]
        shp = tuple(ts[0].shape)
        for k, t in zip(DETAIL_KEYS, ts):
            _check(t, f"detail {k}", contiguous=False)
            if tuple(t.shape) != shp or t.device != x.device:
                raise ValueError(f"waverec3: level {li} detail {k} has shape {tuple(t.shape)}, "
                                 f"expected {shp}")
        if x.dim() != 5 or tuple(x.shape[:2]) != shp[:2] or any(
                a < b or a > b + 1 for a, b in zip(x.shape[2:], shp[2:])):
            raise ValueError(f"waverec3: LL {tuple(x.shape)} does not fit details {shp}")
        x = x[..., :shp[2], :shp[3], :shp[4]]
        B, C, nz, ny, nx = shp
        O = tuple(2 * n - L + 2 for n in shp[2:])
        last = li == nlev - 1
        if last and out is not None:
            if tuple(out.shape) != (B, C) + O or out.stride()[2:] != (O[1] * O[2], O[2], 1):
                raise ValueError(f"waverec3: out {tuple(out.shape)} / {out.stride()} does not "
                                 f"fit ({B},{C})+{O} with a contiguous (z, y, x) block")
            o = out
        else:
            o = torch.empty((B, C) + O, dtype=torch.float32, device=x.device)
        src = [x] + ts
        ptrs = (ctypes.c_void_p * 8)(*[t.data_ptr() for t in src])
        st = (ctypes.c_int64 * 40)(*[s for t in src for s in t.stride()])
        _lib.call("wf_idwt3d_level", ptrs, st, B, C, nz, ny, nx, rlo, rhi, L, o.data_ptr(),
                  o.stride(0), o.stride(1), _stream())
        x = o
    return x


def dwt3d_bwd(gbands: torch.Tensor, size: Sequence[int], wavelet: str) -> torch.Tensor:
    _check(gbands, "gbands", contiguous=False)
    (lo, hi, _, _), L = _filters(wavelet)
    D, H, W = (int(s) for s in size)
    n = tuple((s + L - 1) // 2 for s in (D, H, W))
    if gbands.dim() != 6 or gbands.shape[0] != 8 or tuple(gbands.shape[3:]) != n:
        raise ValueError(f"dwt3d_bwd: expected band gradients (8, B, C) + {n} for an input of "
                         f"{(D, H, W)}, got {tuple(gbands.shape)}")
    gbands = gbands.contiguous()
    B, C = gbands.shape[1:3]
    dx = torch.empty((B, C, D, H, W), dtype=torch.float32, device=gbands.device)
    _lib.call("wf_dwt3d_bwd", gbands.data_ptr(), dx.data_ptr(), B * C, D, H, W, lo, hi, L,
              _stream())
    return dx


def idwt3d_level_bwd(gout: torch.Tensor, ll_size: Sequence[int], wavelet: str,
                     channel_last: Sequence[bool] = (False,) * 8) -> List[torch.Tensor]:
    _check(gout, "gout", contiguous=False)
    (_, _, rlo, rhi), L = _filters(wavelet)
    if gout.dim() != 5:
        raise ValueError(f"idwt3d_level_bwd: expected (B, C, Oz, Oy, Ox), got {tuple(gout.shape)}")
    B, C = gout.shape[:2]
    O = tuple(gout.shape[2:])
    n = tuple((o + L - 2) // 2 for o in O)
    if any(2 * m - L + 2 != o for m, o in zip(n, O)):
        raise ValueError(f"idwt3d_level_bwd: {O} is not the output size of a {L}-tap level")
    ll_size = tuple(int(s) for s in ll_size)
    if len(ll_size) != 3 or any(s < m or s > m + 1 for s, m in zip(ll_size, n)):
        raise ValueError(f"idwt3d_level_bwd: LL size {ll_size} does not fit details {n}")
    if len(channel_last) != 8:
        raise ValueError("idwt3d_level_bwd: channel_last needs one flag per band")
    if not gout[0, 0].is_contiguous():
        gout = gout.contiguous()
    outs = []
    for k in range(8):
        shp = ll_size if k == 0 else n
        if channel_last[k]:
            t = torch.empty((B,) + shp + (C,), dtype=torch.float32,
                            device=gout.device).permute(0, 4, 1, 2, 3)
        else:
            t = torch.empty((B, C) + shp, dtype=torch.float32, device=gout.device)
        outs.append(t)
    ptrs = (ctypes.c_void_p * 8)(*[t.data_ptr() for t in outs])
    st = (ctypes.c_int64 * 40)(*[s for t in outs for s in t.stride()])
    _lib.call("wf_idwt3d_level_bwd", gout.data_ptr(), gout.stride(0), gout.stride(1), B, C,
              n[0], n[1], n[2], ll_size[0] - n[0], ll_size[1] - n[1], ll_size[2] - n[2], rlo, rhi,
              L, ptrs, st, _stream())
    return outs


def cl_ld(x: torch.Tensor) -> Optional[int]:
    if x.dim() != 5:
        return None
    B, C, D, H, W = x.shape
    s = x.stride()
    ld = s[4] if W > 1 else (s[3] if H > 1 else (s[2] if D > 1 else max(C, 1)))
    if (C > 1 and s[1] != 1) or ld < C or ld % 4 or x.data_ptr() % 16:
        return None
    if (W > 1 and s[4] != ld) or (H > 1 and s[3] != W * ld) or (D > 1 and s[2] != H * W * ld):
        return None
    if B > 1 and s[0] != D * H * W * ld:
        return None
    return ld


def resample_trilinear_cf(x: torch.Tensor, size: Sequence[int], dtype=torch.float16,
                          align_corners: bool = False) -> torch.Tensor:
    if x.dim() != 4:
        raise ValueError(f"resample_trilinear_cf: (C, d, h, w) expected, got {tuple(x.shape)}")
    if dtype not in (torch.float16, torch.float32):
        raise TypeError("resample_trilinear_cf: fp16 or fp32 output")
    x = x if x.dtype == torch.float32 else x.float()
    if x.stride()[1:] != (x.shape[2] * x.shape[3], x.shape[3], 1):
        x = x.contiguous()
    _check(x, "x", contiguous=False)
    C, d, h, w = x.shape
    D, H, W = (int(v) for v in size)
    out = torch.empty((C, D, H, W), dtype=dtype, device=x.device)
    _lib.call("wf_resample_trilinear_cf", x.data_ptr(), x.stride(0), C, d, h, w, D, H, W,
              int(bool(align_corners)), out.data_ptr(), int(dtype == torch.float16), _stream())
    return out


def hf_refine(details: Dict[str, torch.Tensor], mod) -> Dict[str, torch.Tensor]:
    ts = [details[k] for k in DETAIL_KEYS]
    B, C, D, H, W = ts[0].shape
    P = D * H * W

    def dense_cl(t):
        st = t.stride()
        return cl_ld(t) == C and st[2:] == (H * W * C, W * C, C)
    ts = [t if dense_cl(t) else t.contiguous(memory_format=torch.channels_last_3d) for t in ts]
    if len({t.stride(0) for t in ts}) != 1:
        ts = [t.contiguous(memory_format=torch.channels_last_3d) for t in ts]
    for t in ts:
        if tuple(t.shape) != (B, C, D, H, W):
            raise ValueError("hf_refine: the 7 detail tensors must share one shape")
        _check(t, "detail", contiguous=False)
    c1, nrm, c2 = mod.conv1, mod.norm, mod.conv2
    for prm, nm in ((c1.weight, "conv1.weight"), (c1.bias, "conv1.bias"), (nrm.weight, "norm.weight"),
                    (nrm.bias, "norm.bias"), (c2.weight, "conv2.weight"), (c2.bias, "conv2.bias")):
        _check(prm, nm)
    out = torch.empty((7, B, D, H, W, C), dtype=torch.float32, device=ts[0].device)
    ws = torch.empty(_lib.query("wf_hf_refine_workspace_bytes", B, C), dtype=torch.uint8,
                     device=out.device)
    ptrs = (ctypes.c_void_p * 7)(*[t.data_ptr() for t in ts])
    _lib.call("wf_hf_refine_fwd", ptrs, ts[0].stride(0), c1.weight.data_ptr(), c1.bias.data_ptr(),
              nrm.weight.data_ptr(), nrm.bias.data_ptr(), float(nrm.eps), c2.weight.data_ptr(),
              c2.bias.data_ptr(), int(mod.sigmoid is not None), out.data_ptr(), ws.data_ptr(),
              B, C, D, H, W, _stream())
    return {k: out[i].permute(0, 4, 1, 2, 3) for i, k in enumerate(DETAIL_KEYS)}


def to_cl(x: torch.Tensor) -> torch.Tensor:
    return x if cl_ld(x) is not None else x.contiguous(memory_format=torch.channels_last_3d)


def _cl_ok(t: torch.Tensor) -> bool:
    return (t.is_cuda and t.dtype == torch.float32 and t.dim() == 5 and t.shape[1] % 4 == 0
            and cl_ld(t) is not None)


def copy_cl(src: torch.Tensor, dst: torch.Tensor) -> torch.Tensor:
    if tuple(src.shape) != tuple(dst.shape):
        raise ValueError(f"copy_cl: shapes {tuple(src.shape)} and {tuple(dst.shape)} differ")
    if not (_cl_ok(src) and _cl_ok(dst)) or src.device != dst.device:
        return dst.copy_(src)
    B, C, D, H, W = src.shape
    _lib.call("wf_copy_cl", src.data_ptr(), cl_ld(src), dst.data_ptr(), cl_ld(dst),
              B * D * H * W, C, _stream())
    return dst


def cat_cl(tensors: Sequence[torch.Tensor]) -> torch.Tensor:
    t0 = tensors[0]
    B, _, D, H, W = t0.shape
    out = empty_cl(B, sum(t.shape[1] for t in tensors), D, H, W, t0.device)
    c = 0
    for t in tensors:
        copy_cl(t, out[:, c:c + t.shape[1]])
        c += t.shape[1]
    return out


def subvoxel_scatter_cl(g: torch.Tensor, bias: Optional[torch.Tensor], dst: torch.Tensor):
    B, _, D2, H2, W2 = dst.shape
    d, h, w = D2 // 2, H2 // 2, W2 // 2
    C = g.shape[1] // 8
    ldd = cl_ld(dst)
    if ldd is None or not g.is_contiguous() or g.shape[0] != B * d * h * w or C % 4:
        raise ValueError("subvoxel_scatter_cl: g must be contiguous (B*d*h*w, 8C), dst channel-last")
    _lib.call("wf_subvoxel_scatter_cl", g.data_ptr(), 0 if bias is None else bias.data_ptr(),
              dst.data_ptr(), ldd, B, C, d, h, w, _stream())
    return dst


def convtranspose2_cl(x: torch.Tensor, weight: torch.Tensor, bias: Optional[torch.Tensor],
                      out: torch.Tensor) -> torch.Tensor:
    B, Cin, d, h, w = x.shape
    if tuple(weight.shape) != (Cin, weight.shape[1], 2, 2, 2):
        raise ValueError(f"convtranspose2_cl: weight {tuple(weight.shape)} does not fit Cin={Cin}")
    Cout = weight.shape[1]
    ldo = cl_ld(out)
    if ldo is None or tuple(out.shape) != (B, out.shape[1], 2 * d, 2 * h, 2 * w) \
            or out.shape[1] < Cout:
        raise ValueError("convtranspose2_cl: out must be a channel-last (B, >=Cout, 2d, 2h, 2w)")
    _check(x, "x", contiguous=False)
    if cl_ld(x) != Cin:
        x = x.contiguous(memory_format=torch.channels_last_3d)
    if bias is not None:
        _check(bias, "bias")

    def make():
        wt = weight.detach().permute(2, 3, 4, 1, 0).reshape(8 * Cout, Cin).contiguous()
        wb = torch.empty((2, 8 * Cout, Cin), dtype=torch.bfloat16, device=wt.device)
        _lib.call("wf_split_f32_to_bf16x2", wt.data_ptr(), wb.data_ptr(), wt.numel(), _stream())
        return wb
    wb = per_forward(("ct2", weight.data_ptr(), tuple(weight.shape)), make)
    _lib.call("wf_convtranspose2_cl", x.data_ptr(), wb.data_ptr(), _ptr(bias), out.data_ptr(),
              ldo, B, Cin, Cout, d, h, w, PRECISIONS["bf16x3"], _stream())
    return out


def cl_parent(t: torch.Tensor, c0: int) -> Optional[torch.Tensor]:
    base = t._base
    if base is None or base.dim() != 5 or cl_ld(base) != base.shape[1] or c0 < 0:
        return None
    if tuple(base.shape[2:]) != tuple(t.shape[2:]) or base.shape[0] != t.shape[0]:
        return None
    if c0 + t.shape[1] > base.shape[1] or cl_ld(t) != base.shape[1]:
        return None
    if t.data_ptr() != base.data_ptr() + c0 * base.element_size():
        return None
    return base


def empty_cl(B: int, C: int, D: int, H: int, W: int, device) -> torch.Tensor:
    return torch.empty((B, C, D, H, W), dtype=torch.float32, device=device,
                       memory_format=torch.channels_last_3d)


def conv3d_k3_packed(weight: torch.Tensor, prec: Optional[int] = None) -> torch.Tensor:
    f16 = (_prec() if prec is None else prec) == FP16

    def make():
        w = weight.detach()
        _check(w, "conv weight", contiguous=False)
        w = w.contiguous()
        Cout, Cin = w.shape[:2]
        n = _lib.query("wf_conv3d_k3_packed_elems", Cin, Cout)
        out = torch.empty(n, dtype=torch.bfloat16, device=w.device)
        _lib.call("wf_conv3d_k3_pack_f16" if f16 else "wf_conv3d_k3_pack", w.data_ptr(),
                  out.data_ptr(), Cin, Cout, _stream())
        return out
    return per_forward(("conv3", weight.data_ptr(), tuple(weight.shape), f16), make)


def _conv3_workspace(B, Cin, Cout, D, H, W, prec, xh, device) -> Optional[torch.Tensor]:
    n = _lib.query("wf_conv3d_k3_workspace_bytes", B, Cin, Cout, D, H, W, prec, int(xh))
    return torch.empty(n, dtype=torch.uint8, device=device) if n > 0 else None


def conv3d_k3(x: torch.Tensor, weight: torch.Tensor, bias: Optional[torch.Tensor] = None,
              out: Optional[torch.Tensor] = None, norm_eps: Optional[float] = None):
    if x.dtype == torch.float16:
        return _conv3d_k3_xh(x, weight, bias, out, norm_eps)
    _check(x, "x", contiguous=False)
    x = to_cl(x)
    B, Cin, D, H, W = x.shape
    Cout = weight.shape[0]
    if tuple(weight.shape) != (Cout, Cin, 3, 3, 3):
        raise ValueError(f"conv3d_k3: weight {tuple(weight.shape)} does not fit Cin={Cin}")
    if bias is not None:
        _check(bias, "bias")
    if out is None:
        out = empty_cl(B, Cout, D, H, W, x.device)
    ldo = cl_ld(out)
    if ldo is None or tuple(out.shape) != (B, Cout, D, H, W):
        raise ValueError("conv3d_k3: out must be a channel-last (B, Cout, D, H, W) tensor")
    acc = None
    if norm_eps is not None:
        acc = torch.zeros((B, Cout, 2), dtype=torch.float64, device=x.device)
    prec = _prec()
    work = _conv3_workspace(B, Cin, Cout, D, H, W, prec, False, x.device)
    _lib.call("wf_conv3d_k3_fwd", x.data_ptr(), cl_ld(x), conv3d_k3_packed(weight, prec).data_ptr(),
              _ptr(bias), out.data_ptr(), ldo, _ptr(acc), _ptr(work), B, Cin, Cout, D, H, W, prec,
              _stream())
    if acc is None:
        return out
    stats = torch.empty((B, 2, Cout), dtype=torch.float32, device=x.device)
    _lib.call("wf_instnorm_finalize", acc.data_ptr(), stats.data_ptr(), B, Cout, D * H * W,
              float(norm_eps), _stream())
    return out, stats


def _conv3d_k3_xh(x, weight, bias, out, norm_eps):
    if _prec() != FP16:
        raise ValueError("conv3d_k3: an fp16 input needs the fp16 precision")
    ld = cl_ld(x)
    if ld is None or not x.is_cuda:
        raise ValueError("conv3d_k3: fp16 input must be a channel-last CUDA tensor")
    B, Cin, D, H, W = x.shape
    Cout = weight.shape[0]
    if tuple(weight.shape) != (Cout, Cin, 3, 3, 3):
        raise ValueError(f"conv3d_k3: weight {tuple(weight.shape)} does not fit Cin={Cin}")
    if bias is not None:
        _check(bias, "bias")
    if out is None:
        out = empty_cl(B, Cout, D, H, W, x.device)
    ldo = cl_ld(out)
    if ldo is None or tuple(out.shape) != (B, Cout, D, H, W):
        raise ValueError("conv3d_k3: out must be a channel-last (B, Cout, D, H, W) tensor")
    acc = None
    if norm_eps is not None:
        acc = torch.zeros((B, Cout, 2), dtype=torch.float64, device=x.device)
    work = _conv3_workspace(B, Cin, Cout, D, H, W, FP16, True, x.device)
    _lib.call("wf_conv3d_k3_fwd_xh", x.data_ptr(), ld, conv3d_k3_packed(weight, FP16).data_ptr(),
              _ptr(bias), out.data_ptr(), ldo, _ptr(acc), _ptr(work), B, Cin, Cout, D, H, W,
              _stream())
    if acc is None:
        return out
    stats = torch.empty((B, 2, Cout), dtype=torch.float32, device=x.device)
    _lib.call("wf_instnorm_finalize", acc.data_ptr(), stats.data_ptr(), B, Cout, D * H * W,
              float(norm_eps), _stream())
    return out, stats


def norm_act_h(a: torch.Tensor, stats_a: torch.Tensor, slope: float = 0.01) -> torch.Tensor:
    lda = cl_ld(a)
    if lda is None:
        raise ValueError("norm_act_h: channel-last input expected")
    B, C, D, H, W = a.shape
    out = torch.empty((B, C, D, H, W), dtype=torch.float16, device=a.device,
                      memory_format=torch.channels_last_3d)
    _lib.call("wf_norm_act_h_cl", a.data_ptr(), lda, stats_a.data_ptr(), out.data_ptr(), C, B, C,
              D * H * W, float(slope), _stream())
    return out


def conv1x1_cl(x: torch.Tensor, weight: torch.Tensor, bias: Optional[torch.Tensor] = None
               ) -> torch.Tensor:
    x = to_cl(x)
    B, Cin, D, H, W = x.shape
    Cout = weight.shape[0]
    if Cin % 8 == 0 and Cout % 4 == 0 and cl_ld(x) == Cin and x.is_cuda:
        rows = x.permute(0, 2, 3, 4, 1).reshape(-1, Cin)
        y = linear_rows(rows, weight, bias, prec=PRECISIONS["bf16x3"])
        return y.view(B, D, H, W, Cout).permute(0, 4, 1, 2, 3)
    rows = x.permute(0, 2, 3, 4, 1).reshape(-1, Cin)
    w2 = weight.reshape(Cout, Cin)
    y = torch.addmm(bias, rows, w2.t()) if bias is not None else torch.mm(rows, w2.t())
    return y.view(B, D, H, W, Cout).permute(0, 4, 1, 2, 3)


def upsample_cl(x: torch.Tensor, size: Sequence[int], align_corners: bool) -> torch.Tensor:
    x = x if (cl_ld(x) == x.shape[1]) else x.contiguous(memory_format=torch.channels_last_3d)
    B, C, d, h, w = x.shape
    D, H, W = size
    out = empty_cl(B, C, D, H, W, x.device)
    _lib.call("wf_upsample_trilinear_cl", x.data_ptr(), out.data_ptr(), B, C, d, h, w, D, H, W,
              int(bool(align_corners)), _stream())
    return out


def upsample_add_cl(x: torch.Tensor, out: torch.Tensor, align_corners: bool) -> torch.Tensor:
    x = x if (cl_ld(x) == x.shape[1]) else x.contiguous(memory_format=torch.channels_last_3d)
    B, C, d, h, w = x.shape
    if cl_ld(out) != C or tuple(out.shape[:2]) != (B, C):
        raise ValueError("upsample_add_cl: out must be a dense channel-last (B, C, D, H, W)")
    D, H, W = out.shape[2:]
    _lib.call("wf_upsample_trilinear_add_cl", x.data_ptr(), out.data_ptr(), B, C, d, h, w, D, H,
              W, int(bool(align_corners)), _stream())
    return out


def conv1x1_head(x: torch.Tensor, weight: torch.Tensor, bias: Optional[torch.Tensor]
                 ) -> torch.Tensor:
    ld = cl_ld(x)
    if ld is None:
        raise ValueError("conv1x1_head: channel-last input expected")
    B, K, D, H, W = x.shape
    N = weight.shape[0]
    w2 = weight.detach().reshape(N, K).contiguous()
    if bias is not None:
        _check(bias, "bias")
    out = torch.empty((B, N, D, H, W), dtype=torch.float32, device=x.device)
    _lib.call("wf_conv1x1_head_cl", x.data_ptr(), ld, w2.data_ptr(), _ptr(bias), out.data_ptr(),
              B, K, N, D * H * W, _stream())
    return out


def dwconv3d_cl(x: torch.Tensor, weight: torch.Tensor, bias: Optional[torch.Tensor],
                norm_eps: Optional[float] = None):
    x = x if (cl_ld(x) == x.shape[1]) else x.contiguous(memory_format=torch.channels_last_3d)
    B, C, D, H, W = x.shape
    if tuple(weight.shape) != (C, 1, 3, 3, 3):
        raise ValueError(f"dwconv3d_cl: weight {tuple(weight.shape)} is not ({C},1,3,3,3)")
    _check(weight, "weight")
    if bias is not None:
        _check(bias, "bias")
    out = empty_cl(B, C, D, H, W, x.device)
    if norm_eps is not None:
        if bias is None or C % 32:
            raise ValueError("dwconv3d_cl: fused statistics need a bias and C % 32 == 0")
        acc = torch.empty((B, C, 2), dtype=torch.float64, device=x.device)
        _lib.call("wf_dwconv3d_stats_cl", x.data_ptr(), weight.data_ptr(), bias.data_ptr(),
                  out.data_ptr(), acc.data_ptr(), B, C, D, H, W, _stream())
        stats = torch.empty((B, 2, C), dtype=torch.float32, device=x.device)
        _lib.call("wf_instnorm_finalize", acc.data_ptr(), stats.data_ptr(), B, C, D * H * W,
                  float(norm_eps), _stream())
        return out, stats
    _lib.call("wf_dwconv3d_cl", x.data_ptr(), weight.data_ptr(), _ptr(bias), 0, out.data_ptr(),
              B, C, D, H, W, _stream())
    return out


def upsample_dwconv3d_cl(x: torch.Tensor, size, weight: torch.Tensor, bias: torch.Tensor,
                         norm_eps: float, align_corners: bool = True):
    x = x if (cl_ld(x) == x.shape[1]) else x.contiguous(memory_format=torch.channels_last_3d)
    B, C, d, h, w = x.shape
    D, H, W = (int(v) for v in size)
    if C % 32 or W < 2 * w or H < 2 * h or bias is None:
        return None
    if tuple(weight.shape) != (C, 1, 3, 3, 3):
        raise ValueError(f"upsample_dwconv3d_cl: weight {tuple(weight.shape)} is not ({C},1,3,3,3)")
    _check(weight, "weight")
    _check(bias, "bias")
    out = empty_cl(B, C, D, H, W, x.device)
    acc = torch.empty((B, C, 2), dtype=torch.float64, device=x.device)
    _lib.call("wf_upsample_dwconv3d_stats_cl", x.data_ptr(), weight.data_ptr(), bias.data_ptr(),
              out.data_ptr(), acc.data_ptr(), B, C, d, h, w, D, H, W, int(bool(align_corners)),
              _stream())
    stats = torch.empty((B, 2, C), dtype=torch.float32, device=x.device)
    _lib.call("wf_instnorm_finalize", acc.data_ptr(), stats.data_ptr(), B, C, D * H * W,
              float(norm_eps), _stream())
    return out, stats


def conv3d_k3_wgrad(x: torch.Tensor, dy: torch.Tensor, wshape) -> torch.Tensor:
    x, dy = to_cl(x), to_cl(dy)
    _check(x, "x", contiguous=False)
    _check(dy, "dy", contiguous=False)
    B, Cin, D, H, W = x.shape
    Cout = dy.shape[1]
    if tuple(wshape) != (Cout, Cin, 3, 3, 3) or tuple(dy.shape) != (B, Cout, D, H, W):
        raise ValueError(f"conv3d_k3_wgrad: x {tuple(x.shape)}, dy {tuple(dy.shape)}, weight "
                         f"{tuple(wshape)} do not match")
    dw = torch.empty(tuple(wshape), dtype=torch.float32, device=x.device)
    ws = torch.empty(_lib.query("wf_conv3d_k3_wgrad_workspace_bytes", B, Cin, Cout, D, H, W),
                     dtype=torch.uint8, device=x.device)
    _lib.call("wf_conv3d_k3_wgrad", x.data_ptr(), cl_ld(x), dy.data_ptr(), cl_ld(dy),
              dw.data_ptr(), 0, ws.data_ptr(), B, Cin, Cout, D, H, W, _stream())
    return dw


def gemm_tn(a: torch.Tensor, b: torch.Tensor, out: Optional[torch.Tensor] = None,
            accumulate: bool = False) -> torch.Tensor:
    if a.dim() != 2 or b.dim() != 2 or a.shape[0] != b.shape[0]:
        raise ValueError(f"gemm_tn: a {tuple(a.shape)} and b {tuple(b.shape)} do not match")
    a = a if a.stride(1) == 1 and a.dtype == torch.float32 else a.float().contiguous()
    b = b if b.stride(1) == 1 and b.dtype == torch.float32 else b.float().contiguous()
    M, N = a.shape
    K = b.shape[1]
    if a.stride(0) < N:
        a = a.contiguous()
    if b.stride(0) < K:
        b = b.contiguous()
    _check(a, "a", contiguous=False)
    _check(b, "b", contiguous=False)
    if b.device != a.device:
        raise ValueError("gemm_tn: a and b must be on the same device")
    if out is None:
        out = torch.empty((N, K), dtype=torch.float32, device=a.device)
        accumulate = False
    if out.dtype != torch.float32 or out.device != a.device:
        raise ValueError(f"gemm_tn: out must be float32 on {a.device}, got {out.dtype} on "
                         f"{out.device}")
    if tuple(out.shape) != (N, K) or out.stride(1) != 1 or out.stride(0) < K:
        raise ValueError("gemm_tn: out must be an (N, K) row matrix")
    ws = torch.empty(max(1, _lib.query("wf_gemm_tn_workspace_bytes", M, N, K)),
                     dtype=torch.uint8, device=a.device)
    _lib.call("wf_gemm_tn", a.data_ptr(), a.stride(0), b.data_ptr(), b.stride(0),
              out.data_ptr(), out.stride(0), int(accumulate), ws.data_ptr(), M, N, K, _stream())
    return out


def linear_rows(x2d: torch.Tensor, weight: torch.Tensor, bias: Optional[torch.Tensor] = None,
                gelu_in: bool = False, cache: bool = True, prec: Optional[int] = None,
                out: Optional[torch.Tensor] = None) -> torch.Tensor:
    _check(x2d, "x")
    M, K = x2d.shape
    N = weight.shape[0]
    w2 = weight.reshape(N, K)
    pr = _prec() if prec is None else prec
    if cache:
        wb = split_weight(weight, (N, K), pr)
    else:
        w2 = w2.contiguous()
        wb = torch.empty((2, N, K), dtype=torch.bfloat16, device=x2d.device)
        _lib.call("wf_cast_f32_to_f16x2" if pr == FP16 else "wf_split_f32_to_bf16x2",
                  w2.data_ptr(), wb.data_ptr(), w2.numel(), _stream())
    if bias is not None:
        _check(bias, "bias")
    if out is None:
        out = torch.empty((M, N), dtype=torch.float32, device=x2d.device)
    elif tuple(out.shape) != (M, N) or not out.is_contiguous() or out.dtype != torch.float32:
        raise ValueError(f"linear_rows: out must be a contiguous fp32 ({M}, {N}) tensor")
    _lib.call("wf_linear_fwd", x2d.data_ptr(), wb.data_ptr(), _ptr(bias), out.data_ptr(), M, K, N,
              int(bool(gelu_in)), pr, _stream())
    return out


def mfma_gemm_ok(a: torch.Tensor, K: int, N: int) -> bool:
    return (a.is_cuda and a.dtype == torch.float32 and a.dim() == 2 and a.is_contiguous()
            and K % 8 == 0 and K >= 8 and N % 4 == 0 and N >= 4)


def smallk_ok(a: torch.Tensor, K: int, N: int) -> bool:
    return (a.is_cuda and a.dtype == torch.float32 and a.dim() == 2 and a.stride(1) == 1
            and 1 <= K <= 7 and N % 4 == 0 and 4 <= N <= 4096)


def linear_smallk(x2d: torch.Tensor, w_nk: torch.Tensor,
                  bias: Optional[torch.Tensor] = None) -> torch.Tensor:
    M, K = x2d.shape
    N = w_nk.shape[0]
    w = w_nk.detach().reshape(N, K).contiguous()
    if x2d.stride(1) != 1 or x2d.stride(0) < K:
        x2d = x2d.contiguous()
    _check(x2d, "x", contiguous=False)
    _check(w, "w")
    if bias is not None:
        bias = bias.detach().contiguous()
        _check(bias, "bias")
    out = torch.empty((M, N), dtype=torch.float32, device=x2d.device)
    _lib.call("wf_linear_smallk_fwd", x2d.data_ptr(), x2d.stride(0), w.data_ptr(),
              _ptr(bias), out.data_ptr(), N, M, K, N, _stream())
    return out


def _rows_dense(a: torch.Tensor) -> torch.Tensor:
    if a.dim() == 2 and a.stride(1) == 1 and not a.is_contiguous():
        return a.contiguous()
    return a


def mm_rows(a: torch.Tensor, b: torch.Tensor) -> torch.Tensor:
    K, N = b.shape
    if smallk_ok(a, K, N):
        return linear_smallk(a, b.t())
    a = _rows_dense(a)
    if not mfma_gemm_ok(a, K, N):
        return a.mm(b)
    return linear_rows(a, b.detach().t().contiguous(), None, cache=False,
                       prec=PRECISIONS["bf16x3"])


def linear_rows_any(x2d: torch.Tensor, weight: torch.Tensor,
                    bias: Optional[torch.Tensor] = None) -> torch.Tensor:
    N, K = weight.shape[0], x2d.shape[1]
    w2 = weight.reshape(N, K)
    if smallk_ok(x2d, K, N):
        return linear_smallk(x2d, w2, bias)
    x2d = _rows_dense(x2d)
    if not mfma_gemm_ok(x2d, K, N):
        return torch.addmm(bias, x2d, w2.t()) if bias is not None else x2d.mm(w2.t())
    return linear_rows(x2d, w2.detach().contiguous(), None if bias is None else bias.detach(),
                       cache=False, prec=PRECISIONS["bf16x3"])


def instnorm_stats(x: torch.Tensor, eps: float) -> torch.Tensor:
    ld = cl_ld(x)
    if ld is None:
        raise ValueError("instnorm_stats: channel-last input expected")
    B, C = x.shape[:2]
    P = x.shape[2] * x.shape[3] * x.shape[4]
    stats = torch.empty((B, 2, C), dtype=torch.float32, device=x.device)
    ws = torch.empty(_lib.query("wf_instnorm_workspace_bytes", B, C), dtype=torch.uint8,
                     device=x.device)
    _lib.call("wf_instnorm_stats_cl", x.data_ptr(), ld, B, C, P, float(eps), stats.data_ptr(),
              ws.data_ptr(), _stream())
    return stats


def norm_act(a: torch.Tensor, stats_a: torch.Tensor, r: Optional[torch.Tensor] = None,
             stats_r: Optional[torch.Tensor] = None, slope: float = 0.01,
             out: Optional[torch.Tensor] = None) -> torch.Tensor:
    lda = cl_ld(a)
    if lda is None:
        raise ValueError("norm_act: channel-last input expected")
    B, C = a.shape[:2]
    P = a.shape[2] * a.shape[3] * a.shape[4]
    ldr = 0
    if r is not None:
        r = to_cl(r)
        if tuple(r.shape) != tuple(a.shape):
            raise ValueError(f"norm_act: residual {tuple(r.shape)} vs {tuple(a.shape)}")
        ldr = cl_ld(r)
    if out is None:
        out = empty_cl(*a.shape, device=a.device)
    ldo = cl_ld(out)
    if ldo is None or tuple(out.shape) != tuple(a.shape):
        raise ValueError("norm_act: out must be channel-last and shaped like a")
    _lib.call("wf_norm_act_cl", a.data_ptr(), lda, stats_a.data_ptr(), _ptr(r), ldr,
              _ptr(stats_r), out.data_ptr(), ldo, B, C, P, float(slope), _stream())
    return out


def norm_act_lin(a: torch.Tensor, stats_a: torch.Tensor, x: torch.Tensor,
                 weight: torch.Tensor, bias: Optional[torch.Tensor], eps: float,
                 slope: float = 0.01, out: Optional[torch.Tensor] = None) -> torch.Tensor:
    lda = cl_ld(a)
    x = to_cl(x)
    ldx = cl_ld(x)
    if lda is None or ldx is None:
        raise ValueError("norm_act_lin: channel-last inputs expected")
    B, C = a.shape[:2]
    K = x.shape[1]
    if not 1 <= K <= 7 or tuple(x.shape[2:]) != tuple(a.shape[2:]) or x.shape[0] != B:
        raise ValueError(f"norm_act_lin: x {tuple(x.shape)} does not fit a {tuple(a.shape)}")
    P = a.shape[2] * a.shape[3] * a.shape[4]
    acc = torch.empty((B, K + K * K), dtype=torch.float64, device=a.device)
    _lib.call("wf_moments_cl", x.data_ptr(), ldx, B, K, P, acc.data_ptr(), _stream())
    mu = acc[:, :K] / P
    cov = acc[:, K:].view(B, K, K) / P - mu[:, :, None] * mu[:, None, :]
    W = weight.detach().reshape(C, K).double()
    bv = bias.detach().double() if bias is not None else torch.zeros(C, dtype=torch.float64,
                                                                     device=a.device)
    mean_r = mu @ W.t() + bv
    var_r = torch.einsum("ck,bkl,cl->bc", W, cov, W).clamp_min(0)
    rstd_r = torch.rsqrt(var_r + eps)
    wfold = (W[None] * rstd_r[..., None]).float().contiguous()
    bfold = ((bv[None] - mean_r) * rstd_r).float().contiguous()
    if out is None:
        out = empty_cl(*a.shape, device=a.device)
    ldo = cl_ld(out)
    if ldo is None or tuple(out.shape) != tuple(a.shape):
        raise ValueError("norm_act_lin: out must be channel-last and shaped like a")
    _lib.call("wf_norm_act_lin_cl", a.data_ptr(), lda, stats_a.data_ptr(), x.data_ptr(), ldx, K,
              wfold.data_ptr(), bfold.data_ptr(), out.data_ptr(), ldo, B, C, P, float(slope),
              _stream())
    return out


def rel_pos_bias(table: torch.Tensor, index: torch.Tensor) -> torch.Tensor:
    _check(table, "relative_position_bias_table")
    _check(index, "relative_position_index", dtype=torch.int64)
    T, heads = table.shape
    N = index.shape[0]
    out = torch.empty((heads, N, N), dtype=torch.float32, device=table.device)
    _lib.call("wf_rel_pos_bias", table.data_ptr(), index.data_ptr(), out.data_ptr(), N, heads, T,
              _stream())
    return out


def index_is_formula(index: torch.Tensor, ws: int) -> bool:
    r = torch.arange(ws)
    s, h, w = torch.meshgrid(r, r, r, indexing="ij")
    pos = torch.stack([s.reshape(-1), h.reshape(-1), w.reshape(-1)], dim=-1)
    d = pos[:, None, :] - pos[None, :, :] + (ws - 1)
    ref = d[..., 0] * (3 * ws - 1) + d[..., 1] * (2 * ws - 1) + d[..., 2]
    return tuple(index.shape) == tuple(ref.shape) and bool(torch.equal(index.detach().cpu(), ref))


def attention_bias(table: torch.Tensor, index: torch.Tensor, ws: int, heads: int,
                   head_dim: int, formula: bool = False) -> torch.Tensor:
    if ws == 8 and head_dim == 16 and formula:
        return table.detach()
    return per_forward(("relbias", table.data_ptr(), index.data_ptr()),
                       lambda: rel_pos_bias(table.detach(), index))


def window_attention(x_cl: torch.Tensor, wqkv: torch.Tensor, bqkv: Optional[torch.Tensor],
                     bias: torch.Tensor, wproj: torch.Tensor, bproj: Optional[torch.Tensor],
                     ws: int, heads: int, scale: float,
                     ln: Optional[Tuple[torch.Tensor, torch.Tensor, float]] = None,
                     prec: Optional[int] = None, more: Sequence[torch.Tensor] = ()):
    _check(x_cl, "x")
    B, D1, H1, W1, C = x_cl.shape
    prec = _prec() if prec is None else prec
    if more:
        return _window_attention_levels((x_cl, *more), wqkv, bqkv, bias, wproj, bproj, ws, heads,
                                        scale, ln, prec)
    wq = split_weight(wqkv, prec=prec)
    wp = split_weight(wproj, prec=prec)
    if bqkv is not None:
        _check(bqkv, "qkv.bias")
    if bproj is not None:
        _check(bproj, "proj.bias")
    _check(bias, "bias")
    N = ws ** 3
    table = tuple(bias.shape) == ((2 * ws - 1) ** 3, heads)
    if not table and tuple(bias.shape) != (heads, N, N):
        raise ValueError(f"window_attention: bias {tuple(bias.shape)} is neither ({heads},{N},{N}) "
                         f"nor the ({(2 * ws - 1) ** 3},{heads}) table")
    lw = lb = None
    eps = 0.0
    if ln is not None:
        lw, lb, eps = ln
    out = torch.empty_like(x_cl)
    prec = _prec() if prec is None else prec
    wsb = _lib.query("wf_window_attention_workspace_bytes", B, C, D1, H1, W1, prec)
    work = torch.empty(wsb, dtype=torch.uint8, device=x_cl.device)
    _lib.call("wf_window_attention_fwd_table" if table else "wf_window_attention_fwd",
              x_cl.data_ptr(), _ptr(lw), _ptr(lb), float(eps),
              wq.data_ptr(), _ptr(bqkv), bias.data_ptr(), wp.data_ptr(), _ptr(bproj),
              out.data_ptr(), work.data_ptr(), B, C, D1, H1, W1, ws, heads, float(scale),
              prec, _stream())
    return out


def _window_attention_levels(levels, wqkv, bqkv, bias, wproj, bproj, ws, heads, scale, ln, prec):
    B, C = levels[0].shape[0], levels[0].shape[4]
    if ln is not None or ws != 8 or tuple(bias.shape) != ((2 * ws - 1) ** 3, heads):
        raise ValueError("window_attention(more=...): the table bias (ws 8, head_dim 16) without "
                         "a LayerNorm only")
    dhw: List[int] = []
    for x in levels:
        _check(x, "x")
        if x.dim() != 5 or x.shape[0] != B or x.shape[4] != C:
            raise ValueError("window_attention(more=...): level batch/channels mismatch")
        dhw.extend(x.shape[1:4])
    for t, name in ((bqkv, "qkv.bias"), (bproj, "proj.bias"), (bias, "bias")):
        if t is not None:
            _check(t, name)
    wq = split_weight(wqkv, prec=prec)
    wp = split_weight(wproj, prec=prec)
    darr = (ctypes.c_int64 * len(dhw))(*dhw)
    wsb = _lib.query("wf_window_attention_levels_workspace_bytes", darr, len(levels), B, C, prec)
    rows = [x.numel() // C for x in levels]
    out = torch.empty((sum(rows), C), dtype=torch.float32, device=levels[0].device)
    work = torch.empty(max(wsb, 0), dtype=torch.uint8, device=out.device)
    arr = (ctypes.c_void_p * len(levels))(*[x.data_ptr() for x in levels])
    _lib.call("wf_window_attention_fwd_levels", arr, darr, len(levels), wq.data_ptr(),
              _ptr(bqkv), bias.data_ptr(), wp.data_ptr(), _ptr(bproj), out.data_ptr(),
              work.data_ptr(), B, C, heads, float(scale), prec, _stream())
    views = LevelViews(o.view(x.shape) for o, x in zip(out.split(rows), levels))
    views.buffer = out
    return views


class LevelViews(tuple):
    """window_attention(more=...)'s result: the per-level views, and as `.buffer` the one
    (sum of rows, C) tensor they are views of."""


def msfuse(srcs: Sequence[torch.Tensor], shortcut: torch.Tensor, ln_eps: Optional[float],
           branch_scale: Optional[torch.Tensor] = None
           ) -> Tuple[torch.Tensor, Optional[torch.Tensor]]:
    _check(shortcut, "shortcut")
    B, D, H, W, C = shortcut.shape
    if len(srcs) > 4:
        raise ValueError("msfuse: at most 4 sources")
    dhw: List[int] = []
    for s in srcs:
        _check(s, "src")
        if s.shape[0] != B or s.shape[4] != C:
            raise ValueError("msfuse: source batch/channels mismatch")
        dhw.extend(s.shape[1:4])
    out = torch.empty_like(shortcut)
    stats = None
    if ln_eps is not None:
        stats = torch.empty((B * D * H * W, 2), dtype=torch.float32, device=shortcut.device)
    arr = (ctypes.c_void_p * max(1, len(srcs)))(*[s.data_ptr() for s in srcs])
    darr = (ctypes.c_int64 * max(1, len(dhw)))(*dhw)
    if branch_scale is not None:
        _check(branch_scale, "branch_scale")
    _lib.call("wf_msfuse_fwd", arr, darr, len(srcs), shortcut.data_ptr(), _ptr(branch_scale),
              out.data_ptr(),
              _ptr(stats), float(ln_eps or 0.0), B, C, D, H, W, _stream())
    return out, stats


def ccf_ffn(xh: torch.Tensor, stats: Optional[torch.Tensor], norm2: Optional[torch.nn.Module],
            mlp: torch.nn.Module, branch_scale: Optional[torch.Tensor] = None) -> torch.Tensor:
    n2w = n2b = None
    if stats is not None:
        n2w, n2b = norm2.weight, norm2.bias
    return ccf_ffn_raw(xh, stats, n2w, n2b, mlp.pwconv.weight, mlp.pwconv.bias,
                       mlp.norm1.weight, mlp.norm1.bias, float(mlp.norm1.eps),
                       mlp.dwconv.weight, mlp.dwconv.bias, mlp.norm2.weight, mlp.norm2.bias,
                       float(mlp.norm2.eps), mlp.fc.weight, mlp.fc.bias, branch_scale)


def ccf_ffn_raw(xh, stats, n2w, n2b, pww, pwb, l1w, l1b, eps1, dww, dwb, l2w, l2b, eps2, fcw, fcb,
                branch_scale=None, prec: Optional[int] = None) -> torch.Tensor:
    _check(xh, "x")
    B, D, H, W, C = xh.shape
    hid = pww.shape[0]
    prec = _prec() if prec is None else prec
    pw = split_weight(pww, (hid, C), prec)
    fc = split_weight(fcw, prec=prec)
    out = torch.empty_like(xh)
    wsb = _lib.query("wf_ccf_ffn_workspace_bytes", B, C, hid, D, H, W, prec)
    work = torch.empty(wsb, dtype=torch.uint8, device=xh.device)
    args = (xh.data_ptr(), _ptr(stats), _ptr(n2w), _ptr(n2b),
            pw.data_ptr(), _ptr(pwb), l1w.data_ptr(), l1b.data_ptr(), float(eps1),
            dww.data_ptr(), dwb.data_ptr(), l2w.data_ptr(), l2b.data_ptr(), float(eps2),
            fc.data_ptr(), _ptr(fcb), _ptr(branch_scale),
            out.data_ptr(), work.data_ptr(), B, C, hid, D, H, W, prec, _stream())
    ccf_ffn_pwconv(args)
    ccf_ffn_dwconv(args, B * D * H * W, hid)
    ccf_ffn_fc(args)
    return out


def ccf_ffn_pwconv(args):
    _lib.call("wf_ccf_ffn_stage", 1, *args)


def ccf_ffn_dwconv(args, positions: int, hidden: int):
    _lib.call("wf_ccf_ffn_stage", 2, *args)


def ccf_ffn_fc(args):
    _lib.call("wf_ccf_ffn_stage", 3, *args)


def patch_merging(x_cl: torch.Tensor, norm: torch.nn.LayerNorm, reduction: torch.nn.Linear,
                  v2: bool = False) -> torch.Tensor:
    return _patch_merging_raw(x_cl, norm.weight, norm.bias, float(norm.eps), reduction.weight,
                              v2, _prec())


def _patch_merging_raw(x_cl, ln_w, ln_b, eps, red_w, v2, prec) -> torch.Tensor:
    _check(x_cl, "x")
    B, D, H, W, C = x_cl.shape
    red = split_weight(red_w, prec=prec)
    out = torch.empty((B, D // 2, H // 2, W // 2, 2 * C), dtype=torch.float32, device=x_cl.device)
    _lib.call("wf_patch_merging_fwd", x_cl.data_ptr(), ln_w.data_ptr(), ln_b.data_ptr(),
              float(eps), red.data_ptr(), int(bool(v2)), out.data_ptr(), B, C, D, H, W, prec,
              _stream())
    return out


BLEND_MODES = {"constant": 0, "gaussian": 1}


def importance_map(roi: Sequence[int], mode: str = "constant",
                   sigma_scale: Sequence[float] = (0.125, 0.125, 0.125),
                   device: Optional[torch.device] = None) -> torch.Tensor:
    if mode not in BLEND_MODES:
        raise ValueError(f"Unsupported mode: {mode}, available options are {sorted(BLEND_MODES)}.")
    rd, rh, rw = (int(v) for v in roi)
    device = torch.device(device) if device is not None else torch.device(
        "cuda", torch.cuda.current_device())
    if device.type != "cuda":
        raise RuntimeError("importance_map: GPU only")
    out = torch.empty((rd, rh, rw), dtype=torch.float32, device=device)
    sig = (ctypes.c_float * 3)(*[float(s) for s in sigma_scale])
    _lib.call("wf_importance_map", BLEND_MODES[mode], sig, out.data_ptr(), rd, rh, rw, _stream())
    return out


def sliding_window_stitch(patches: torch.Tensor, weight_map: torch.Tensor,
                          starts: Sequence[Sequence[int]], image_size: Sequence[int],
                          batch: int, world: int = 1, slots_per_round: int = 1) -> torch.Tensor:
    _check(patches, "patches")
    _check(weight_map, "importance_map")
    rows, C = patches.shape[:2]
    roi = tuple(patches.shape[2:])
    if tuple(weight_map.shape) != roi:
        raise ValueError(f"sliding_window_stitch: map {tuple(weight_map.shape)} != roi {roi}")
    nwin = [len(s) for s in starts]
    total = batch * nwin[0] * nwin[1] * nwin[2]
    slots = -(-total // world)
    slots = -(-slots // slots_per_round) * slots_per_round
    if rows < slots * world:
        raise ValueError(f"sliding_window_stitch: {rows} patch rows < {slots * world} needed")
    D, H, W = (int(v) for v in image_size)
    out = torch.empty((batch, C, D, H, W), dtype=torch.float32, device=patches.device)
    flat = [int(s) for ax in starts for s in ax]
    sarr = (ctypes.c_int64 * len(flat))(*flat)
    narr = (ctypes.c_int64 * 3)(*nwin)
    _lib.call("wf_sliding_window_stitch", patches.data_ptr(), int(world), int(slots_per_round),
              weight_map.data_ptr(), sarr, narr, out.data_ptr(), batch, C, D, H, W, *roi,
              _stream())
    return out


def sliding_window_stitch_partial(patches: torch.Tensor, weight_map: torch.Tensor,
                                  starts: Sequence[Sequence[int]], image_size: Sequence[int],
                                  batch: int, world: int, rank: int) -> torch.Tensor:
    _check(patches, "patches")
    _check(weight_map, "importance_map")
    rows, C = patches.shape[:2]
    roi = tuple(patches.shape[2:])
    if tuple(weight_map.shape) != roi:
        raise ValueError(f"sliding_window_stitch_partial: map {tuple(weight_map.shape)} != roi {roi}")
    nwin = [len(s) for s in starts]
    total = batch * nwin[0] * nwin[1] * nwin[2]
    if rows < -(-total // world):
        raise ValueError(f"sliding_window_stitch_partial: {rows} rows < {-(-total // world)}")
    D, H, W = (int(v) for v in image_size)
    out = torch.empty((batch, C + 1, D, H, W), dtype=torch.float32, device=patches.device)
    flat = [int(s) for ax in starts for s in ax]
    _lib.call("wf_sliding_window_stitch_partial", patches.data_ptr(), int(world), int(rank),
              weight_map.data_ptr(), (ctypes.c_int64 * len(flat))(*flat),
              (ctypes.c_int64 * 3)(*nwin), out.data_ptr(), batch, C, D, H, W, *roi, _stream())
    return out


def sliding_window_normalize(num: torch.Tensor) -> torch.Tensor:
    _check(num, "num")
    B, C1, D, H, W = num.shape
    out = torch.empty((B, C1 - 1, D, H, W), dtype=torch.float32, device=num.device)
    _lib.call("wf_sliding_window_normalize", num.data_ptr(), out.data_ptr(), B, C1 - 1, D, H, W,
              _stream())
    return out


def tta_merge(pred: torch.Tensor, passes: Sequence[Sequence[int]]) -> torch.Tensor:
    _check(pred, "pred")
    P, C, D, H, W = pred.shape
    if len(passes) != P:
        raise ValueError(f"tta_merge: {len(passes)} passes for {P} predictions")
    masks = [sum(1 << (d - 2) for d in f) for f in passes]
    out = torch.empty((1, C, D, H, W), dtype=torch.float32, device=pred.device)
    _lib.call("wf_tta_merge", pred.data_ptr(), (ctypes.c_int * P)(*masks), P, out.data_ptr(),
              C, D, H, W, _stream())
    return out


def proj_out(x_cl: torch.Tensor, normalize: bool, eps: float = 1e-5) -> torch.Tensor:
    _check(x_cl, "x")
    B, D, H, W, C = x_cl.shape
    out = torch.empty((B, C, D, H, W), dtype=torch.float32, device=x_cl.device)
    _lib.call("wf_proj_out_fwd", x_cl.data_ptr(), out.data_ptr(), int(bool(normalize)),
              float(eps), B, C, D * H * W, _stream())
    return out


def proj_out_cl(x_cl: torch.Tensor, normalize: bool, eps: float = 1e-5) -> torch.Tensor:
    _check(x_cl, "x")
    B, D, H, W, C = x_cl.shape
    out = torch.empty_like(x_cl)
    if normalize:
        _lib.call("wf_proj_out_cl_fwd", x_cl.data_ptr(), out.data_ptr(), float(eps),
                  B * D * H * W, C, _stream())
    else:
        out.copy_(x_cl)
    return out.permute(0, 4, 1, 2, 3)
```

Before: 1251 volumes/s.

## Compute q/k/v projections inside the windowed attention core kernel

Adds a fused attention kernel that computes the K and V projections for a window straight from the fp32 level inputs into LDS, and computes Q per tile in registers, instead of first running a separate QKV GEMM that writes the qkv buffer to global memory. A rule enables it for C=48 when windows×heads is large enough, and a mode argument can force the staged or fused path. This removes one kernel launch and the qkv write and read-back, in exchange for repeating projection work across q-splits and adding register pressure inside the attention kernel.

```diff
diff --git a/include/waveformer_hip.h b/include/waveformer_hip.h
--- a/include/waveformer_hip.h
+++ b/include/waveformer_hip.h
@@ -7,7 +7,7 @@
 extern "C" {
 #endif
 
-#define WF_ABI_VERSION 20
+#define WF_ABI_VERSION 21
 
 enum { WF_PREC_BF16 = 0, WF_PREC_BF16X3 = 1, WF_PREC_FP16 = 2 };
 
@@ -194,6 +194,14 @@
                                    const float* bproj, float* out, void* workspace, int64_t B,
                                    int64_t C, int64_t heads, float scale, int precision,
                                    void* stream);
+int wf_window_attention_fwd_levels_mode(const float* const* x, const int64_t* dhw, int nlev,
+                                        const uint16_t* wqkv_bf16x2, const float* bqkv,
+                                        const float* table, const uint16_t* wproj_bf16x2,
+                                        const float* bproj, float* out, void* workspace,
+                                        int64_t B, int64_t C, int64_t heads, float scale,
+                                        int precision, void* stream, int qkv_mode);
+int wf_window_attention_levels_fused(const int64_t* dhw, int nlev, int64_t B, int64_t C,
+                                     int64_t heads, int precision);
 
 int wf_msfuse_fwd(const float* const* src, const int64_t* src_dhw, int nsrc,
                   const float* shortcut, const float* branch_scale, float* out, float* stats,
diff --git a/waveformer_amd/_lib.py b/waveformer_amd/_lib.py
--- a/waveformer_amd/_lib.py
+++ b/waveformer_amd/_lib.py
@@ -83,6 +83,9 @@
     "wf_window_attention_levels_workspace_bytes": (_I64, [_P, _I, _I64, _I64, _I]),
     "wf_window_attention_fwd_levels": (_I, [_P, _P, _I, _P, _P, _P, _P, _P, _P, _P, _I64, _I64,
                                             _I64, _F, _I, _P]),
+    "wf_window_attention_fwd_levels_mode": (_I, [_P, _P, _I, _P, _P, _P, _P, _P, _P, _P, _I64,
+                                                 _I64, _I64, _F, _I, _P, _I]),
+    "wf_window_attention_levels_fused": (_I, [_P, _I, _I64, _I64, _I64, _I]),
     "wf_msfuse_fwd": (_I, [_P, _P, _I, _P, _P, _P, _P, _F, _I64, _I64, _I64, _I64, _I64, _P]),
     "wf_ccf_ffn_workspace_bytes": (_I64, [_I64, _I64, _I64, _I64, _I64, _I64, _I]),
     "wf_ccf_ffn_fwd": (_I, [_P, _P, _P, _P, _P, _P, _P, _P, _F, _P, _P, _P, _P, _F, _P, _P,
@@ -130,7 +133,7 @@
     "wf_transpose_cs": (_I, [_P, _P, _I64, _I64, _I64, _P]),
 }
 
-ABI_VERSION = 20
+ABI_VERSION = 21
 _lock = threading.Lock()
 _lib = None
 _err = None
diff --git a/waveformer_amd/csrc/attention.hip b/waveformer_amd/csrc/attention.hip
--- a/waveformer_amd/csrc/attention.hip
+++ b/waveformer_amd/csrc/attention.hip
@@ -1,5 +1,5 @@
 #include "attn_levels.hpp"
-#include "kernels.hpp"
+#include "gemm_common.hpp"
 
 namespace wf {
 
@@ -231,8 +231,171 @@
 constexpr float kTau = 16.0f;
 }
 
-template <int P, int NQ>
-__device__ __forceinline__ void attn_tbl_tiles(const void* __restrict__ qkv, void* __restrict__ out,
+template <int CW>
+struct FusedQkv {
+  static constexpr int NKS = (CW + 31) / 32;
+};
+
+template <int P, int CW>
+__device__ __forceinline__ f32x4 fused_tile(const float (&v)[FusedQkv<CW>::NKS][8],
+                                            const bf16x8 (&wh)[FusedQkv<CW>::NKS],
+                                            const bf16x8 (&wl)[FusedQkv<CW>::NKS], int g4) {
+  f32x4 acc = f32x4{0, 0, 0, 0};
+#pragma unroll
+  for (int ks = 0; ks < FusedQkv<CW>::NKS; ++ks) {
+    const int k = ks * 32 + 8 * g4;
+    float x[8];
+#pragma unroll
+    for (int j = 0; j < 8; ++j) x[j] = v[ks][j];
+    bf16x8 ah, al;
+    a_fragment<P>(x, 0.f, 1.f, nullptr, nullptr, k, k < CW, false, false, ah, al);
+    acc = mma3<P>(acc, wh[ks], wl[ks], ah, al);
+  }
+  return acc;
+}
+template <int P, int CW>
+__device__ __forceinline__ void fused_load_w(const GemmArgs& g, int wo, int g4,
+                                             bf16x8 (&wh)[FusedQkv<CW>::NKS],
+                                             bf16x8 (&wl)[FusedQkv<CW>::NKS]) {
+#pragma unroll
+  for (int ks = 0; ks < FusedQkv<CW>::NKS; ++ks) {
+    const int off = wo + min(ks * 32 + 8 * g4, CW - 8);
+    wh[ks] = *reinterpret_cast<const bf16x8*>(g.w + off);
+    wl[ks] = P == PREC_SPLIT ? *reinterpret_cast<const bf16x8*>(g.w + 3 * CW * CW + off) : wh[ks];
+  }
+}
+struct WindowRows {
+  const float* corner;
+  int H, W;
+  __device__ __forceinline__ WindowRows() : corner(nullptr), H(0), W(0) {}
+  __device__ __forceinline__ WindowRows(const GemmArgs& g, int row0) {
+    row0 = __builtin_amdgcn_readfirstlane(row0);
+    const int l = (row0 >= g.lv_row0[1]) + (row0 >= g.lv_row0[2]) + (row0 >= g.lv_row0[3]);
+    const int r0 = l == 0 ? g.lv_row0[0] : l == 1 ? g.lv_row0[1] : l == 2 ? g.lv_row0[2] : g.lv_row0[3];
+    const int mD = l == 0 ? g.lv_D[0] : l == 1 ? g.lv_D[1] : l == 2 ? g.lv_D[2] : g.lv_D[3];
+    const int mH = l == 0 ? g.lv_H[0] : l == 1 ? g.lv_H[1] : l == 2 ? g.lv_H[2] : g.lv_H[3];
+    const int mW = l == 0 ? g.lv_W[0] : l == 1 ? g.lv_W[1] : l == 2 ? g.lv_W[2] : g.lv_W[3];
+    const float* src = l == 0 ? g.lv_src[0] : l == 1 ? g.lv_src[1] : l == 2 ? g.lv_src[2] : g.lv_src[3];
+    H = mH;
+    W = mW;
+    corner = src + (int64_t)window_row_pos(row0 - r0, 8, mD, mH, mW) * g.K;
+  }
+  __device__ __forceinline__ int64_t row(int t, int K) const {
+    return (int64_t)(((t >> 6) * H + ((t >> 3) & 7)) * W + (t & 7)) * K;
+  }
+};
+template <int CW>
+__device__ __forceinline__ void fused_load_x(const WindowRows& w, int t, int g4,
+                                             float (&v)[FusedQkv<CW>::NKS][8]) {
+  const int64_t off = w.row(t, CW);
+#pragma unroll
+  for (int ks = 0; ks < FusedQkv<CW>::NKS; ++ks)
+    load8f<false>(w.corner, off + min(ks * 32 + 8 * g4, CW - 8), v[ks]);
+}
+
+template <int P, int CW, bool DOK, bool DOV>
+__device__ __forceinline__ void fused_stage_pass(const GemmArgs& g, const WindowRows& w, int h,
+                                                 uint16_t* Ks, uint16_t* Vq) {
+  using namespace tbl;
+  constexpr int NKS = FusedQkv<CW>::NKS;
+  constexpr bool SPLIT = P == PREC_SPLIT;
+  const int lane = threadIdx.x & 63, wid = threadIdx.x >> 6;
+  const int l15 = lane & 15, g4 = lane >> 4;
+  bf16x8 kwh[NKS], kwl[NKS], vwh[NKS], vwl[NKS];
+  if (DOK) fused_load_w<P, CW>(g, (CW + h * HD + l15) * CW, g4, kwh, kwl);
+  if (DOV) fused_load_w<P, CW>(g, (2 * CW + h * HD + l15) * CW, g4, vwh, vwl);
+  f32x4 kb = f32x4{0, 0, 0, 0}, vb = kb;
+  if (g.bias) {
+    if (DOK) kb = *reinterpret_cast<const f32x4*>(g.bias + CW + h * HD + 4 * g4);
+    if (DOV) vb = *reinterpret_cast<const f32x4*>(g.bias + 2 * CW + h * HD + 4 * g4);
+  }
+  constexpr int DEPTH = CW <= 48 ? 4 : 2;
+  float v[DEPTH][NKS][8];
+#pragma unroll
+  for (int tt = 0; tt < DEPTH; ++tt) fused_load_x<CW>(w, wid * 64 + tt * 16 + l15, g4, v[tt]);
+#pragma unroll
+  for (int tt = 0; tt < 4; ++tt) {
+    const int key = wid * 64 + tt * 16 + l15;
+    f32x4 ka = f32x4{0, 0, 0, 0}, va = ka;
+    if (DOK) ka = fused_tile<P, CW>(v[tt % DEPTH], kwh, kwl, g4);
+    if (DOV) va = fused_tile<P, CW>(v[tt % DEPTH], vwh, vwl, g4);
+    if (tt + DEPTH < 4) fused_load_x<CW>(w, key + 16 * DEPTH, g4, v[tt % DEPTH]);
+    if (g.bias) {
+      ka += kb;
+      va += vb;
+    }
+    if (DOK) {
+      bf16x4 kh, kl;
+      split4<P>(ka, kh, kl);
+      const int sw = kswz(key), hc = g4 >> 1, ho = 4 * (g4 & 1);
+      *reinterpret_cast<bf16x4*>(&Ks[key * KS + 8 * (hc ^ sw) + ho]) = kh;
+      *reinterpret_cast<bf16x4*>(&Ks[key * KS + 8 * ((2 + hc) ^ sw) + ho]) =
+          SPLIT ? kl : bf16x4{0, 0, 0, 0};
+    }
+    if (DOV) {
+      bf16x4 vh, vl;
+      split4<P>(va, vh, vl);
+      const int vo = (key >> 2) * VB + (4 * g4) * 4 + (key & 3);
+#pragma unroll
+      for (int i = 0; i < 4; ++i) {
+        Vq[vo + 4 * i] = (uint16_t)vh[i];
+        if (SPLIT) Vq[VQ + vo + 4 * i] = (uint16_t)vl[i];
+      }
+    }
+  }
+}
+template <int P, int CW>
+__device__ __forceinline__ void fused_stage_kv(const GemmArgs& g, int row0, int h, uint16_t* Ks,
+                                               uint16_t* Vq) {
+  const WindowRows w(g, row0);
+  if constexpr (CW <= 48) {
+    fused_stage_pass<P, CW, true, true>(g, w, h, Ks, Vq);
+  } else {
+    fused_stage_pass<P, CW, true, false>(g, w, h, Ks, Vq);
+    fused_stage_pass<P, CW, false, true>(g, w, h, Ks, Vq);
+  }
+}
+
+template <int P, int CW>
+__device__ __forceinline__ void fused_q_operands(const GemmArgs& g, const WindowRows& w, int t,
+                                                 int h, float sc, bf16x8& hi, bf16x8& lo) {
+  using namespace tbl;
+  constexpr int NKS = FusedQkv<CW>::NKS;
+  const int lane = threadIdx.x & 63, l15 = lane & 15, g4 = lane >> 4;
+  int wo = (h * HD + l15) * CW;
+  asm volatile("" : "+v"(wo));
+  bf16x8 wh[NKS], wl[NKS];
+  fused_load_w<P, CW>(g, wo, g4, wh, wl);
+  float v[NKS][8];
+  fused_load_x<CW>(w, t, g4, v);
+  f32x4 q = fused_tile<P, CW>(v, wh, wl, g4);
+  if (g.bias) q += *reinterpret_cast<const f32x4*>(g.bias + h * HD + 4 * g4);
+  bf16x4 qh, ql;
+  if (store32(P)) {
+    const f32x4 a = q * sc;
+#pragma unroll
+    for (int i = 0; i < 4; ++i) {
+      const uint16_t hh = op_cvt<P>(a[i]);
+      qh[i] = (short)hh;
+      ql[i] = op_lo<P>(a[i], hh);
+    }
+  } else {
+#pragma unroll
+    for (int i = 0; i < 4; ++i) qh[i] = (short)f2bf(bf2f(f2bf(q[i])) * sc);
+    ql = bf16x4{0, 0, 0, 0};
+  }
+  const u32x2 hw = __builtin_bit_cast(u32x2, qh), lw = __builtin_bit_cast(u32x2, ql);
+  const int sa = l15 + 32 * (g4 & 1), sb = sa + 16;
+  hi = __builtin_bit_cast(bf16x8, u32x4{(uint32_t)__shfl((int)hw[0], sa, 64), (uint32_t)__shfl((int)hw[1], sa, 64),
+                                        (uint32_t)__shfl((int)hw[0], sb, 64), (uint32_t)__shfl((int)hw[1], sb, 64)});
+  if (P == PREC_SPLIT)
+    lo = __builtin_bit_cast(bf16x8, u32x4{(uint32_t)__shfl((int)lw[0], sa, 64), (uint32_t)__shfl((int)lw[1], sa, 64),
+                                          (uint32_t)__shfl((int)lw[0], sb, 64), (uint32_t)__shfl((int)lw[1], sb, 64)});
+}
+
+template <int P, int NQ, int CW = 0>
+__device__ __forceinline__ void attn_tbl_tiles(const void* __restrict__ qkv,
+                                               const GemmArgs* __restrict__ g, void* __restrict__ out,
                                                const f32x4* tq, const uint16_t* Ks,
                                                const uint16_t* Vq, int64_t row0, int q0, int h,
                                                int heads, int nsub, float scale_log2) {
@@ -246,6 +409,7 @@
   const bf16x8 z8 = {0, 0, 0, 0, 0, 0, 0, 0};
   const short one = (short)op_cvt<P>(1.0f);
   const bf16x8 ones = bf16x8{one, one, one, one, one, one, one, one};
+  const WindowRows wrows = CW != 0 ? WindowRows(*g, (int)row0) : WindowRows();
   for (int st = wid; st < nsub; st += 8 * NQ) {
     int qq[NQ], rbq[NQ];
     bf16x8 b1[NQ], b2[NQ];
@@ -256,7 +420,10 @@
       const int q = q0 + (st + 8 * u) * 16 + l15;
       qq[u] = q;
       bf16x8 hi = z8, lo = z8;
-      load8_split_scaled<P>(qkv, (row0 + q) * ld + h * HD + 8 * (g4 & 1), scale_log2, hi, lo);
+      if constexpr (CW != 0)
+        fused_q_operands<P, CW>(*g, wrows, q, h, scale_log2, hi, lo);
+      else
+        load8_split_scaled<P>(qkv, (row0 + q) * ld + h * HD + 8 * (g4 & 1), scale_log2, hi, lo);
       b1[u] = hi;
       b2[u] = (SPLIT && g4 < 2) ? lo : z8;
       const int qz = q >> 6, qy = (q >> 3) & 7, qx = q & 7;
@@ -359,6 +526,20 @@
         *reinterpret_cast<bf16x4*>(reinterpret_cast<uint16_t*>(out) + off) = r;
       }
     }
+  }
+}
+
+__device__ __forceinline__ void attn_tbl_stage_table(f32x4* tq, const float* __restrict__ table,
+                                                     int heads, int h) {
+  using namespace tbl;
+  for (int i = threadIdx.x; i < TBLN; i += 512) {
+    const float v = table[(int64_t)i * heads + h] * 1.4426950408889634f;
+    const int j = TBLN - 1 - i;
+#pragma unroll
+    for (int c = 0; c < 4; ++c)
+      if (j - c >= 0) reinterpret_cast<float*>(&tq[j - c])[c] = v;
+    if (j >= TBLN - 3)
+      for (int c = TBLN - j; c < 4; ++c) reinterpret_cast<float*>(&tq[j])[c] = 0.f;
   }
 }
 
@@ -382,15 +563,7 @@
   const int64_t row0 = bw * N;
   const bf16x8 z8 = {0, 0, 0, 0, 0, 0, 0, 0};
 
-  for (int i = tid; i < TBLN; i += 512) {
-    const float v = table[(int64_t)i * heads + h] * 1.4426950408889634f;
-    const int j = TBLN - 1 - i;
-#pragma unroll
-    for (int c = 0; c < 4; ++c)
-      if (j - c >= 0) reinterpret_cast<float*>(&tq[j - c])[c] = v;
-    if (j >= TBLN - 3)
-      for (int c = TBLN - j; c < 4; ++c) reinterpret_cast<float*>(&tq[j])[c] = 0.f;
-  }
+  attn_tbl_stage_table(tq, table, heads, h);
   for (int it = tid; it < N * 2; it += 512) {
     const int key = it >> 1, ch = it & 1, sw = kswz(key);
     bf16x8 hi = z8, lo = z8;
@@ -419,16 +592,43 @@
   const int nsub = N / 16 / qsplit;
   const int q0 = qs * (N / qsplit);
   if (nsub >= 16 && bw < pair_end)
-    attn_tbl_tiles<P, 2>(qkv, out, tq, Ks, Vq, row0, q0, h, heads, nsub, scale_log2);
+    attn_tbl_tiles<P, 2>(qkv, nullptr, out, tq, Ks, Vq, row0, q0, h, heads, nsub, scale_log2);
   else
-    attn_tbl_tiles<P, 1>(qkv, out, tq, Ks, Vq, row0, q0, h, heads, nsub, scale_log2);
-}
-
-bool attn_tbl_pair_loop(int64_t wh) { return wh >= 256; }
+    attn_tbl_tiles<P, 1>(qkv, nullptr, out, tq, Ks, Vq, row0, q0, h, heads, nsub, scale_log2);
+}
+
+template <int P, int CW>
+__global__ __launch_bounds__(512) __attribute__((amdgpu_waves_per_eu(4, 4))) void attn_tbl_kernel_fused(const GemmArgs g,
+                                                                const float* __restrict__ table,
+                                                                void* __restrict__ out, int heads,
+                                                                int qsplit, float scale_log2,
+                                                                int64_t pair_end) {
+  using namespace tbl;
+  __shared__ __attribute__((aligned(16))) uint8_t lds_tbl[TQ_BYTES + N * KS * 2 + 2 * VQ * 2];
+  f32x4* tq = reinterpret_cast<f32x4*>(lds_tbl);
+  uint16_t* Ks = reinterpret_cast<uint16_t*>(lds_tbl + TQ_BYTES);
+  uint16_t* Vq = Ks + N * KS;
+  int qs, h;
+  int64_t bw;
+  attn_block(qsplit, heads, qs, h, bw);
+  const int64_t row0 = bw * N;
+  attn_tbl_stage_table(tq, table, heads, h);
+  fused_stage_kv<P, CW>(g, (int)row0, h, Ks, Vq);
+  __syncthreads();
+
+  const int nsub = N / 16 / qsplit;
+  const int q0 = qs * (N / qsplit);
+  if (nsub >= 16 && bw < pair_end)
+    attn_tbl_tiles<P, 2, CW>(nullptr, &g, out, tq, Ks, Vq, row0, q0, h, heads, nsub, scale_log2);
+  else
+    attn_tbl_tiles<P, 1, CW>(nullptr, &g, out, tq, Ks, Vq, row0, q0, h, heads, nsub, scale_log2);
+}
+
+bool attn_tbl_pair_loop(int64_t wh) { return wh >= kAttnPairLoopWH; }
 
 int launch_attn_core(const void* qkv, const float* bias, void* out, float* lse, int64_t Bw,
                      int N, int heads, int hd, float scale, int prec, hipStream_t s,
-                     int table_ws, int64_t pair_windows) {
+                     int table_ws, int64_t pair_windows, const GemmArgs* fused) {
   if (Bw <= 0) return WF_OK;
   const int64_t nblk = cdiv(N, kQB) * heads * Bw;
   if (nblk > 0x7fffffff) return fail(WF_E_SHAPE, "attention: too many (window, head) tiles");
@@ -447,6 +647,20 @@
     auto k = split ? attn_tbl_kernel<PREC_SPLIT>
                    : (f16 ? attn_tbl_kernel<PREC_FP16> : attn_tbl_kernel<PREC_BF16>);
     const int64_t pair_end = pair_windows < 0 ? Bw : pair_windows;
+    if (fused) {
+      void (*kf)(GemmArgs, const float*, void*, int, int, float, int64_t) = nullptr;
+#define ATTN_FUSED_CASE(CWV)                                                               \
+  if (fused->K == CWV)                                                                     \
+    kf = split ? attn_tbl_kernel_fused<PREC_SPLIT, CWV>                                    \
+               : (f16 ? attn_tbl_kernel_fused<PREC_FP16, CWV> : attn_tbl_kernel_fused<PREC_BF16, CWV>);
+      ATTN_FUSED_CASE(48)
+      ATTN_FUSED_CASE(96)
+#undef ATTN_FUSED_CASE
+      if (!kf || !gemm_levels_callsite(*fused) || fused->N != 3 * fused->K || heads * 16 != fused->K)
+        return fail(WF_E_SHAPE, "attention core (q/k/v in the core): instantiated for C = 48 and 96");
+      hipLaunchKernelGGL(kf, g1, dim3(512), 0, s, *fused, bias, out, heads, qsplit, sl2, pair_end);
+      return check_launch("attention core (table bias, q/k/v in the core)");
+    }
     hipLaunchKernelGGL(k, g1, dim3(512), 0, s, qkv, bias, out, heads, qsplit, sl2, pair_end);
     return check_launch("attention core (table bias, window per workgroup)");
   }
@@ -523,6 +737,28 @@
   return g;
 }
 
+static void set_level_sources(GemmArgs& g, const float* const* x, const AttnLevels& L) {
+  g.a_map = MAP_LEVELS;
+  for (int l = 0; l < WF_MAX_LEVELS; ++l) {
+    const bool on = l < L.nlev;
+    g.lv_src[l] = on ? x[l] : x[0];
+    g.lv_row0[l] = on ? (int)L.row0[l] : 0x7fffffff;
+    g.lv_D[l] = on ? L.D[l] : kAttnLevelsWs;
+    g.lv_H[l] = on ? L.H[l] : kAttnLevelsWs;
+    g.lv_W[l] = on ? L.W[l] : kAttnLevelsWs;
+  }
+}
+
+static int pick_qkv_fused(int qkv_mode, int64_t windows, int64_t heads, int64_t C) {
+  if (qkv_mode == ATTN_QKV_STAGED) return 0;
+  if (qkv_mode == ATTN_QKV_FUSED) {
+    if (!attn_qkv_fused_width(C))
+      return fail(WF_E_SHAPE, "window attention: q/k/v in the core is instantiated for C = 48 and 96");
+    return 1;
+  }
+  return attn_qkv_fused(windows, heads, C) ? 1 : 0;
+}
+
 static GemmArgs proj_gemm_args(const void* ao, const uint16_t* wproj, const float* bproj,
                                float* out, int64_t rows, int64_t C, int prec) {
   GemmArgs p{};
@@ -572,7 +808,8 @@
                                  const uint16_t* wproj_bf16x2, const float* bproj, float* out,
                                  void* workspace, float* lse, int64_t B, int64_t C, int64_t D1,
                                  int64_t H1, int64_t W1, int64_t ws, int64_t heads, float scale,
-                                 int precision, void* stream) {
+                                 int precision, void* stream,
+                                 int qkv_mode = ATTN_QKV_STAGED) {
   WF_REQUIRE(B >= 1 && C >= 8 && C % 8 == 0, "C must be a positive multiple of 8");
   WF_REQUIRE(ws >= 1 && D1 % ws == 0 && H1 % ws == 0 && W1 % ws == 0,
              "the raster must tile into ws^3 windows (window_partition, wave_helper.py:459)");
@@ -591,6 +828,28 @@
   hipStream_t s = (hipStream_t)stream;
   void* qkv = workspace;
   void* ao = reinterpret_cast<char*>(workspace) + attn_workspace(rows, C, precision).ao;
+  if (table_ws == kAttnLevelsWs && !ln_w && !lse && C == 16 * heads && rows <= 0x7fffffff &&
+      reinterpret_cast<uintptr_t>(x) % 16 == 0) {
+    const int fused = pick_qkv_fused(qkv_mode, Bw, heads, C);
+    if (fused < 0) return WF_E_SHAPE;
+    if (fused) {
+      const int64_t dhw[3] = {D1, H1, W1};
+      AttnLevels L;
+      if (const char* why = attn_levels_plan(dhw, 1, B, C, heads, L))
+        return fail(WF_E_SHAPE, std::string("window attention: ") + why);
+      GemmArgs g = qkv_gemm_args(x, nullptr, nullptr, 0.f, wqkv_bf16x2, bqkv, qkv, rows, B, C, 0, 0,
+                                 0, ws, precision);
+      set_level_sources(g, &x, L);
+      const int rc = launch_attn_core(nullptr, bias, ao, nullptr, Bw, (int)N, (int)heads, 16, scale,
+                                      precision, s, table_ws, -1, &g);
+      if (rc) return rc;
+      return launch_gemm(proj_gemm_args(ao, wproj_bf16x2, bproj, out, rows, C, precision), s,
+                         "wf_window_attention_fwd(proj)");
+    }
+  } else if (qkv_mode == ATTN_QKV_FUSED) {
+    return fail(WF_E_SHAPE, "window attention: q/k/v in the core needs the table bias (ws 8, "
+                            "head_dim 16), inference, no LayerNorm in the loader");
+  }
   int rc = launch_gemm(qkv_gemm_args(x, ln_w, ln_b, ln_eps, wqkv_bf16x2, bqkv, qkv, rows, B, C,
                                      D1, H1, W1, ws, precision),
                        s, "wf_window_attention_fwd(qkv)");
@@ -627,7 +886,7 @@
              "table-bias attention is implemented for window 8 and head_dim 16");
   return window_attention_impl(x, ln_w, ln_b, ln_eps, wqkv_bf16x2, bqkv, table, (int)ws,
                                wproj_bf16x2, bproj, out, workspace, nullptr, B, C, D1, H1, W1,
-                               ws, heads, scale, precision, stream);
+                               ws, heads, scale, precision, stream, ATTN_QKV_RULE);
 }
 
 extern "C" int wf_window_attention_fwd(const float* x, const float* ln_w, const float* ln_b,
@@ -650,12 +909,33 @@
   return attn_workspace(L.row0[nlev], C, precision).bytes;
 }
 
+extern "C" int wf_window_attention_levels_fused(const int64_t* dhw, int nlev, int64_t B, int64_t C,
+                                               int64_t heads, int precision) {
+  AttnLevels L;
+  if (!valid_prec(precision) || attn_levels_plan(dhw, nlev, B, C, heads, L)) return 0;
+  return attn_qkv_fused(L.row0[nlev] / (kAttnLevelsWs * kAttnLevelsWs * kAttnLevelsWs), heads, C) ? 1 : 0;
+}
+
 extern "C" int wf_window_attention_fwd_levels(const float* const* x, const int64_t* dhw, int nlev,
                                               const uint16_t* wqkv_bf16x2, const float* bqkv,
                                               const float* table, const uint16_t* wproj_bf16x2,
                                               const float* bproj, float* out, void* workspace,
                                               int64_t B, int64_t C, int64_t heads, float scale,
                                               int precision, void* stream) {
+  return wf_window_attention_fwd_levels_mode(x, dhw, nlev, wqkv_bf16x2, bqkv, table, wproj_bf16x2,
+                                             bproj, out, workspace, B, C, heads, scale, precision,
+                                             stream, ATTN_QKV_RULE);
+}
+
+extern "C" int wf_window_attention_fwd_levels_mode(const float* const* x, const int64_t* dhw,
+                                                   int nlev, const uint16_t* wqkv_bf16x2,
+                                                   const float* bqkv, const float* table,
+                                                   const uint16_t* wproj_bf16x2,
+                                                   const float* bproj, float* out, void* workspace,
+                                                   int64_t B, int64_t C, int64_t heads, float scale,
+                                                   int precision, void* stream, int qkv_mode) {
+  WF_REQUIRE(qkv_mode >= ATTN_QKV_RULE && qkv_mode <= ATTN_QKV_FUSED,
+             "qkv_mode: -1 (the rule), 0 (staged) or 1 (q/k/v in the core)");
   AttnLevels L;
   if (const char* why = attn_levels_plan(dhw, nlev, B, C, heads, L))
     return fail(WF_E_SHAPE, std::string(__func__) + ": " + why);
@@ -675,17 +955,11 @@
   hipStream_t s = (hipStream_t)stream;
   void* qkv = workspace;
   void* ao = reinterpret_cast<char*>(workspace) + attn_workspace(rows, C, precision).ao;
+  const int fused = pick_qkv_fused(qkv_mode, rows / N, heads, C);
+  if (fused < 0) return WF_E_SHAPE;
   GemmArgs g = qkv_gemm_args(x[0], nullptr, nullptr, 0.f, wqkv_bf16x2, bqkv, qkv, rows, B, C, 0,
                              0, 0, ws, precision);
-  g.a_map = MAP_LEVELS;
-  for (int l = 0; l < WF_MAX_LEVELS; ++l) {
-    const bool on = l < nlev;
-    g.lv_src[l] = on ? x[l] : x[0];
-    g.lv_row0[l] = on ? (int)L.row0[l] : 0x7fffffff;
-    g.lv_D[l] = on ? L.D[l] : (int)ws;
-    g.lv_H[l] = on ? L.H[l] : (int)ws;
-    g.lv_W[l] = on ? L.W[l] : (int)ws;
-  }
+  set_level_sources(g, x, L);
   int64_t pair_windows = 0;
   bool prefix = true;
   for (int l = 0; l < nlev; ++l) {
@@ -695,20 +969,20 @@
       pair_windows = L.row0[l + 1] / N;
     }
   }
-  if (!prefix || (!try_launch_gemm_rows(g, s, true) && !try_launch_gemm_kc(g, s))) {
+  if (!prefix || (!fused && !try_launch_gemm_rows(g, s, true) && !try_launch_gemm_kc(g, s))) {
     for (int l = 0; l < nlev; ++l) {
       const int rc = window_attention_impl(x[l], nullptr, nullptr, 0.f, wqkv_bf16x2, bqkv, table,
                                            (int)ws, wproj_bf16x2, bproj, out + L.row0[l] * C,
                                            workspace, nullptr, B, C, L.D[l], L.H[l], L.W[l], ws,
-                                           heads, scale, precision, stream);
+                                           heads, scale, precision, stream, qkv_mode);
       if (rc) return rc;
     }
     return WF_OK;
   }
-  int rc = check_launch("wf_window_attention_fwd_levels(qkv)");
+  int rc = fused ? WF_OK : check_launch("wf_window_attention_fwd_levels(qkv)");
   if (rc) return rc;
   rc = launch_attn_core(qkv, table, ao, nullptr, rows / N, (int)N, (int)heads, 16, scale,
-                        precision, s, (int)ws, pair_windows);
+                        precision, s, (int)ws, pair_windows, fused ? &g : nullptr);
   if (rc) return rc;
   return launch_gemm(proj_gemm_args(ao, wproj_bf16x2, bproj, out, rows, C, precision), s,
                      "wf_window_attention_fwd_levels(proj)");
diff --git a/waveformer_amd/csrc/attn_levels.hpp b/waveformer_amd/csrc/attn_levels.hpp
--- a/waveformer_amd/csrc/attn_levels.hpp
+++ b/waveformer_amd/csrc/attn_levels.hpp
@@ -36,4 +36,14 @@
   return nullptr;
 }
 
+constexpr int64_t kAttnPairLoopWH = 256;
+
+enum AttnQkvMode { ATTN_QKV_RULE = -1, ATTN_QKV_STAGED = 0, ATTN_QKV_FUSED = 1 };
+
+inline bool attn_qkv_fused_width(int64_t C) { return C == 48 || C == 96; }
+
+inline bool attn_qkv_fused(int64_t windows, int64_t heads, int64_t C) {
+  return C == 48 && windows * heads >= kAttnPairLoopWH;
 }
+
+}
diff --git a/waveformer_amd/csrc/kernels.hpp b/waveformer_amd/csrc/kernels.hpp
--- a/waveformer_amd/csrc/kernels.hpp
+++ b/waveformer_amd/csrc/kernels.hpp
@@ -133,7 +133,7 @@
 
 int launch_attn_core(const void* qkv, const float* bias, void* out, float* lse, int64_t Bw,
                      int N, int heads, int hd, float scale, int prec, hipStream_t s,
-                     int table_ws = 0, int64_t pair_windows = -1);
+                     int table_ws = 0, int64_t pair_windows = -1, const GemmArgs* fused = nullptr);
 bool attn_tbl_pair_loop(int64_t wh);
 
 int launch_dwconv_ln_gelu(const void* in, const float* w, const float* b, const float* ln_w,
diff --git a/waveformer_amd/ops.py b/waveformer_amd/ops.py
--- a/waveformer_amd/ops.py
+++ b/waveformer_amd/ops.py
@@ -1172,13 +1172,15 @@
                      bias: torch.Tensor, wproj: torch.Tensor, bproj: Optional[torch.Tensor],
                      ws: int, heads: int, scale: float,
                      ln: Optional[Tuple[torch.Tensor, torch.Tensor, float]] = None,
-                     prec: Optional[int] = None, more: Sequence[torch.Tensor] = ()):
+                     prec: Optional[int] = None, more: Sequence[torch.Tensor] = (),
+                     qkv_mode: int = -1):
     _check(x_cl, "x")
     B, D1, H1, W1, C = x_cl.shape
     prec = _prec() if prec is None else prec
-    if more:
-        return _window_attention_levels((x_cl, *more), wqkv, bqkv, bias, wproj, bproj, ws, heads,
-                                        scale, ln, prec)
+    if more or qkv_mode != -1:
+        out = _window_attention_levels((x_cl, *more), wqkv, bqkv, bias, wproj, bproj, ws, heads,
+                                       scale, ln, prec, qkv_mode)
+        return out if more else out[0]
     wq = split_weight(wqkv, prec=prec)
     wp = split_weight(wproj, prec=prec)
     if bqkv is not None:
@@ -1207,7 +1209,8 @@
     return out
 
 
-def _window_attention_levels(levels, wqkv, bqkv, bias, wproj, bproj, ws, heads, scale, ln, prec):
+def _window_attention_levels(levels, wqkv, bqkv, bias, wproj, bproj, ws, heads, scale, ln, prec,
+                             qkv_mode=-1):
     B, C = levels[0].shape[0], levels[0].shape[4]
     if ln is not None or ws != 8 or tuple(bias.shape) != ((2 * ws - 1) ** 3, heads):
         raise ValueError("window_attention(more=...): the table bias (ws 8, head_dim 16) without "
@@ -1229,9 +1232,9 @@
     out = torch.empty((sum(rows), C), dtype=torch.float32, device=levels[0].device)
     work = torch.empty(max(wsb, 0), dtype=torch.uint8, device=out.device)
     arr = (ctypes.c_void_p * len(levels))(*[x.data_ptr() for x in levels])
-    _lib.call("wf_window_attention_fwd_levels", arr, darr, len(levels), wq.data_ptr(),
+    _lib.call("wf_window_attention_fwd_levels_mode", arr, darr, len(levels), wq.data_ptr(),
               _ptr(bqkv), bias.data_ptr(), wp.data_ptr(), _ptr(bproj), out.data_ptr(),
-              work.data_ptr(), B, C, heads, float(scale), prec, _stream())
+              work.data_ptr(), B, C, heads, float(scale), prec, _stream(), int(qkv_mode))
     views = LevelViews(o.view(x.shape) for o, x in zip(out.split(rows), levels))
     views.buffer = out
     return views
```

After: 1266 volumes/s, median of 6. 1.01x the previous value.
